# oss0430/SRFRD

Measured on NVIDIA B200. Metric: training seqs/sec; full-catalogue top-10 users/sec, higher is better.
Workload: dtype bf16

## Files before the change

include/srfrd_b200.h:

```cpp
#ifndef SRFRD_B200_H
#define SRFRD_B200_H

#include <stddef.h>
#include <stdint.h>

#ifdef __cplusplus
extern "C" {
#endif

#define SRFRD_ABI_VERSION 10
#if defined(__GNUC__)
#define SRFRD_API __attribute__((visibility("default")))
#else
#define SRFRD_API
#endif

SRFRD_API const char* srfrd_last_error(void);
SRFRD_API int srfrd_abi_version(void);
SRFRD_API int srfrd_device_check(void);

SRFRD_API int srfrd_embed_ln_fwd(const float* item_table, int64_t n_rows, int D, const float* pos_table,
                       const float* aux_table, int64_t n_aux, int F, int mode, const int64_t* seq,
                       const int64_t* aux_ids, int64_t B, int L, float item_scale, const float* ln_w,
                       const float* ln_b, float eps, void* x0_bf16, float* x0_f32, void* q_bf16, float* stats,
                       int ldx, float drop_p, uint64_t drop_seed, uint32_t drop_stream, const float* drop_step,
                       void* stream);

SRFRD_API int srfrd_srfu_labels(const int64_t* fake_ids, int64_t B, int L, int kind, int64_t* labels, void* stream);

SRFRD_API int srfrd_embed_bwd(const void* dx0_bf16, int ldx, const int64_t* seq, const int64_t* aux_ids, int64_t B, int L,
                    int D, int F, int mode, float item_scale, float* d_item, float* d_aux, void* stream);

SRFRD_API int srfrd_layernorm_fwd(const void* x_bf16, int ldx, const float* w, const float* b, float eps, void* y_bf16,
                        float* y_f32, int ldy, float* stats, int64_t T, int H, int64_t row_stride,
                        int64_t row_offset, void* stream);
SRFRD_API int srfrd_layernorm_bwd(const void* dy_bf16, const float* dy_f32, int lddy, const void* x_bf16, int ldx,
                        const float* stats, const float* w, const void* add_bf16, int ldadd,
                        const int64_t* row_ids, void* dx_bf16, int lddx, float* dw, float* db, int64_t T, int H,
                        void* stream);

typedef struct {
  const float* bias;
  const void* residual;
  const void* gate;
  const int64_t* row_ids;
  void* out_bf16;
  float* out_f32;
  int ldr, ldg, ldc;
  int relu;
  float drop_p;
  uint32_t drop_stream;
  uint64_t drop_seed;
  const float* drop_step;
  void* ln_out_bf16;
  const float* ln_w;
  const float* ln_b;
  float* ln_stats;
  int ld_ln;
  float ln_eps;
} srfrd_gemm_epilogue_t;

SRFRD_API int srfrd_gemm_tn(const void* A_bf16, int lda, const void* B_bf16, int ldb, int M, int N, int K,
                  const srfrd_gemm_epilogue_t* ep, void* stream);
SRFRD_API int srfrd_gemm_tn_plan(int M, int N, int K, int has_aux, int bf16_out, int fused_ln, int* out);
SRFRD_API int srfrd_gemm_debug_read(long long* host_dst);
SRFRD_API int srfrd_attn_debug_read(long long* host_dst);

SRFRD_API int srfrd_gemm_wgrad(const void* dY_bf16, int lda, const void* X_bf16, int ldb, int64_t T, int Mo, int No,
                     float* dW, int ldw, float* dbias, void* stream);
SRFRD_API int srfrd_gemm_ref(const void* A, int lda, const void* B, int ldb, float* C, int ldc, int M, int N, int K,
                   int a_mn_major, int b_mn_major, void* stream);

SRFRD_API int srfrd_colsum(const void* X_bf16, int64_t M, int N, int64_t ld, float* out, void* stream);
SRFRD_API int srfrd_add_segments(float* in, int64_t n, int seg_in, int seg_out, float* out, void* stream);

SRFRD_API int srfrd_dropout_apply(const void* x_bf16, int ldx, void* out_bf16, int ldo, int64_t M, int N, float drop_p,
                        uint64_t seed, uint32_t stream_id, const float* drop_step, void* stream);

typedef struct {
  const float* src; int src_ld;
  void* dst; int dst_ld;
  void* dst_t; int dst_t_ld;
  int rows, cols;
  int dst_is_f32;
} srfrd_cast_desc_t;
SRFRD_API int srfrd_cast_weights(const srfrd_cast_desc_t* descs_dev, int n, void* stream);
SRFRD_API int srfrd_f32_to_bf16_split(const float* src, int64_t src_ld, const int64_t* row_index, void* hi, void* lo,
                            int64_t rows, int cols, int dst_ld, void* stream);

SRFRD_API int srfrd_attention_fwd(const void* q, int ldq, const void* k, const void* v, int ldkv, void* o, int ldo,
                        float* stats, int64_t B, int L, int H, int heads, float drop_p, uint64_t seed, uint32_t stream_id,
                        const float* drop_step, void* stream);
SRFRD_API int srfrd_attention_bwd(const void* dout, int lddo, const void* q, int ldq, const void* k, const void* v, int ldkv,
                        const void* o, int ldo, float* stats, void* dq, int lddq, void* dk, void* dv, int lddkv, int64_t B,
                        int L, int H, int heads, float drop_p, uint64_t seed, uint32_t stream_id, const float* drop_step,
                        void* stream);

SRFRD_API int srfrd_score_fwd(const float* h, int ldh, const float* item_table, const float* fake_table, const int64_t* pos,
                    const int64_t* neg, const int64_t* prs, const int64_t* nrs, int64_t T, int D, int F, float* zp,
                    float* zn, void* stream);
SRFRD_API int srfrd_score_bwd(const float* h, int ldh, const float* item_table, const float* fake_table, const int64_t* pos,
                    const int64_t* neg, const int64_t* prs, const int64_t* nrs, const float* dzp, const float* dzn,
                    int64_t T, int D, int F, float* dh, int lddh, float* d_item, float* d_fake, void* stream);
SRFRD_API int srfrd_score_loss_fused(const float* h, int ldh, const float* item_table, const float* fake_table,
                           const int64_t* pos, const int64_t* neg, const int64_t* prs, const int64_t* nrs,
                           const float* w_pos, const float* w_neg, const float* norm, int64_t T, int D, int F,
                           float* zp, float* zn, float* loss_acc, float* dh, int lddh, float* d_item, float* d_fake,
                           void* stream);
SRFRD_API int srfrd_weight_sums(const int64_t* pos, const float* w_pos, const float* w_neg, int64_t T, float* out2,
                      void* stream);
SRFRD_API int srfrd_loss_finalize(float* acc2, const float* norm2, float* loss, void* stream);

SRFRD_API int srfrd_adam_tick(float* state3, float beta1, float beta2, void* stream);
SRFRD_API int srfrd_adam_step(float* p, float* g, float* m, float* v, int64_t n, float lr, float beta1, float beta2, float eps,
                    const float* state3, int zero_grad, void* stream);

SRFRD_API int srfrd_adam_step_fused(float* p, float* g, float* m, float* v, int64_t n, float lr, float beta1, float beta2,
                          float eps, float* state8, int zero_grad, float* acc2, const float* norm2, float* loss,
                          void* stream, const int64_t* l2_seg, int l2_n_seg, const float* l2_coef, const float* l2_reg);

SRFRD_API int srfrd_param_l2_plan(const int64_t* seg_host, int n_seg, int64_t* n_chunks);
SRFRD_API int srfrd_param_l2(const float* p, const int64_t* seg, int n_seg, int64_t n_chunks, float l2, float* coef,
                   float* reg, double* ws, void* stream);

#define SRFRD_TOPK_KMAX 64
SRFRD_API int srfrd_catalogue_topk_plan(int64_t U, int64_t n_rows, int64_t row_lo, int D, int n_split, int* chunks_out,
                                        int k);
SRFRD_API int srfrd_catalogue_topk_kmax(int D, int n_split, int* kmax_out);
SRFRD_API int srfrd_catalogue_topk(const void* feats_bf16, int64_t U, int64_t u_pad, int n_split, const void* table_bf16,
                         int64_t n_rows, int64_t row_lo, int64_t id_base, int D, int ld_feats, int ld_table,
                         int chunks, float* part_scores, int* part_ids, float* packed_out, void* stream, int k);
SRFRD_API int srfrd_merge_topk(const float* scores, const int* ids, int64_t U, int nlists, int k, float* out_scores,
                     int64_t* out_ids, void* stream);
SRFRD_API int srfrd_merge_topk_packed(const float* packed, int64_t U, int nlists, int k, float* out_scores,
                            int64_t* out_ids, void* stream);
SRFRD_API int srfrd_catalogue_rank(const void* feats_bf16, int64_t U, int64_t u_pad, int n_split,
                                   const void* table_bf16, int64_t n_rows, int64_t row_lo, int64_t id_base,
                                   int D, int ld_feats, int ld_table,
                                   const void* target_rows_bf16, int ld_target, const int64_t* target_ids,
                                   float* target_scores, int* rank_out, void* stream);

SRFRD_API int srfrd_catalogue_ce_plan(int Dp, int64_t* smem_bytes, int* ring_stages, int* tmem_cols);
SRFRD_API int srfrd_catalogue_ce_fwd(const void* h_bf16, int ldh, const void* table_bf16, int ldt, int64_t n_items, int Dp,
                                     const int64_t* pos, const float* w_pos, const int* row_tok, const int* rows_dev,
                                     int64_t cap_rows, float* lse, float* loss_acc, void* stream);
SRFRD_API int srfrd_catalogue_ce_bwd(const void* h_bf16, int ldh, const void* table_bf16, int ldt, int64_t n_items, int Dp,
                                     int D, const int64_t* pos, const float* w_pos, const float* norm, const int* row_tok,
                                     const int* rows_dev, int64_t cap_rows, const float* lse, float* dh, int lddh,
                                     float* d_item, int ldd, void* stream);

SRFRD_API int srfrd_sample_batch(const int64_t* offsets, const int* items, const int8_t* labels, const float* p_fake,
                       const int* eligible, int n_eligible, int itemnum, int B, int L, int policy, uint64_t seed,
                       const float* step, int64_t* users, int64_t* seq, int64_t* rsq, int64_t* pos, int64_t* prs,
                       int64_t* neg, int64_t* nrs, float* w_pos, void* stream);

SRFRD_API int srfrd_sample_candidates(const int64_t* offsets, const int* items, const int* users0, const int* target,
                            int64_t U, int itemnum, int C, uint64_t seed, int64_t* cand, void* stream);
SRFRD_API int srfrd_candidate_rank(const float* feats, int ldf, const float* item_table, int64_t n_rows, int D,
                         const int64_t* cand, int64_t U, int C, const float* fake_table, int F,
                         const int64_t* user_label, float* logits, int ldl, int* rank, int* err_flag, void* stream);
SRFRD_API int srfrd_add_user_term(float* logits, int ldl, int64_t U, int I, const float* feats_tail, int ldf,
                        const float* fake_table, const int64_t* label, int F, void* stream);

typedef struct {
  int* rows;
  int* cnt;
  int* seq_first;
  int* tok_row;
  int* row_tok;
  int64_t* row_ids;
  int* row_info;
  int* tile_row0;
  int* last_row;
  int64_t cap;
} srfrd_pack_t;
SRFRD_API int srfrd_pack_plan(const int64_t* seq, const int64_t* keep, int64_t B, int L, const srfrd_pack_t* pk, void* stream);
SRFRD_API int srfrd_set_row_limit(const int* rows_dev);
SRFRD_API int srfrd_embed_ln_fwd_packed(const float* item_table, int64_t n_rows, int D, const float* pos_table,
                              const float* aux_table, int64_t n_aux, int F, int mode, const int64_t* seq,
                              const int64_t* aux_ids, int64_t B, int L, float item_scale, const float* ln_w,
                              const float* ln_b, float eps, void* x0_bf16, void* q_bf16, float* stats, int ldx,
                              float drop_p, uint64_t drop_seed, uint32_t drop_stream, const float* drop_step,
                              const int* row_tok, const int* rows_dev, int64_t cap_rows, void* stream);
SRFRD_API int srfrd_layernorm_fwd_rows(const void* x_bf16, int ldx, const float* w, const float* b, float eps, float* y_f32,
                             int ldy, const int* row_index, int64_t n, int H, void* stream);
SRFRD_API int srfrd_attention_packed_supported(int L, int H, int heads);
SRFRD_API int srfrd_attention_packed_oproj_supported(int L, int H, int heads);
SRFRD_API int srfrd_attention_fwd_packed(const void* q, int ldq, const void* k, const void* v, int ldkv, void* o, int ldo,
                               const srfrd_pack_t* pk, int L, int H, int heads, float drop_p, uint64_t seed,
                               uint32_t stream_id, const float* drop_step, void* stream, const void* wo, int ldw,
                               const float* bo, const void* res, int ldres, const float* ln_w, const float* ln_b,
                               float ln_eps, float* ln_stats, void* r, int ldr, void* y, int ldy);
SRFRD_API int srfrd_attention_bwd_packed(const void* dout, int lddo, const void* q, int ldq, const void* k, const void* v,
                               int ldkv, void* dq, int lddq, void* dk, void* dv, int lddkv, const srfrd_pack_t* pk,
                               int L, int H, int heads, float drop_p, uint64_t seed, uint32_t stream_id,
                               const float* drop_step, void* stream, const void* dr, int lddr, const void* woT, int ldw);
SRFRD_API int srfrd_score_loss_fused_packed(const float* h, int ldh, const float* item_table, const float* fake_table,
                                  const int64_t* pos, const int64_t* neg, const int64_t* prs, const int64_t* nrs,
                                  const float* w_pos, const float* w_neg, const float* norm, int D, int F,
                                  float* loss_acc, float* dh, int lddh, float* d_item, float* d_fake,
                                  const int* row_tok, const int* rows_dev, int64_t cap_rows, void* stream);
SRFRD_API int srfrd_embed_bwd_packed(const void* dx0_bf16, int ldx, const int64_t* seq, const int64_t* aux_ids,
                           const int* row_tok, const int* rows_dev, int64_t cap_rows, int L, int D, int F, int mode,
                           float item_scale, float* d_item, float* d_aux, float* d_pos, void* stream);

typedef struct {
  const float* bias1; const float* bias2;
  const void* gate; int ldg;
  int relu1;
  float drop1_p, drop2_p; uint32_t drop1_stream, drop2_stream; uint64_t drop_seed; const float* drop_step;
  const void* residual; int ldr;
  int residual_is_a;
  const int64_t* row_ids;
  void* mid_out; int ldm;
  void* out; int ldc;
  void* ln_out; int ld_ln; const float* ln_w; const float* ln_b; float* ln_stats; float ln_eps;
} srfrd_mlp2_t;
SRFRD_API int srfrd_mlp2_tn(const void* A_bf16, int lda, const void* W1_bf16, int ldw1, const void* W2_bf16, int ldw2, int M, int N,
                  const srfrd_mlp2_t* ep, void* stream);

SRFRD_API int srfrd_attention_live_items(const int* tok_row, int64_t B, int L, int heads, int* q_lo, int* items, int* n_live,
                               void* stream);
SRFRD_API int srfrd_set_attention_live(const int* q_lo, const int* items, const int* n_live, const int* tok_row);

typedef struct {
  const void* src; int ld_s;
  void* dst; int ld_d;
  int W;
  int mode;
} srfrd_repack_part_t;
SRFRD_API int srfrd_unpack_rows(const srfrd_repack_part_t* parts, int n_parts, const srfrd_pack_t* pk, int64_t B, int L,
                      void* stream);
SRFRD_API int srfrd_pack_rows(const srfrd_repack_part_t* parts, int n_parts, const srfrd_pack_t* pk, int64_t B, int L,
                    void* stream);

SRFRD_API int srfrd_dp_adam_step(float* const* grad_ptrs_dev, float* const* param_ptrs_dev, uint32_t* const* signal_ptrs_dev,
                       int rank, int world, int64_t n, float* m, float* v, float lr, float beta1, float beta2, float eps,
                       float* state8, const float* norm2, uint32_t* local4, void* stream, const int64_t* l2_seg,
                       int l2_n_seg, const float* l2_coef, const float* l2_reg);

#ifdef __cplusplus
}
#endif
#endif
```

srfrd_b200/_lib.py:

```python
from __future__ import annotations

import ctypes as C
import os

_HERE = os.path.dirname(os.path.abspath(__file__))
LIB_PATH = os.environ.get("SRFRD_B200_LIB") or os.path.join(_HERE, "lib", "libsrfrd_b200.so")

vp, i32, i64, f32, u32, u64 = C.c_void_p, C.c_int, C.c_int64, C.c_float, C.c_uint32, C.c_uint64


class GemmEpilogue(C.Structure):
    _fields_ = [("bias", vp), ("residual", vp), ("gate", vp), ("row_ids", vp), ("out_bf16", vp), ("out_f32", vp),
                ("ldr", i32), ("ldg", i32), ("ldc", i32), ("relu", i32), ("drop_p", f32), ("drop_stream", u32),
                ("drop_seed", u64), ("drop_step", vp),
                ("ln_out_bf16", vp), ("ln_w", vp), ("ln_b", vp), ("ln_stats", vp), ("ld_ln", i32), ("ln_eps", f32)]


class CastDesc(C.Structure):
    _fields_ = [("src", vp), ("src_ld", i32), ("dst", vp), ("dst_ld", i32), ("dst_t", vp), ("dst_t_ld", i32),
                ("rows", i32), ("cols", i32), ("dst_is_f32", i32)]


class Mlp2Epilogue(C.Structure):
    _fields_ = [("bias1", vp), ("bias2", vp), ("gate", vp), ("ldg", i32), ("relu1", i32), ("drop1_p", f32), ("drop2_p", f32),
                ("drop1_stream", u32), ("drop2_stream", u32), ("drop_seed", u64), ("drop_step", vp), ("residual", vp), ("ldr", i32),
                ("residual_is_a", i32), ("row_ids", vp), ("mid_out", vp), ("ldm", i32), ("out", vp), ("ldc", i32),
                ("ln_out", vp), ("ld_ln", i32), ("ln_w", vp), ("ln_b", vp), ("ln_stats", vp), ("ln_eps", f32)]


class PackDesc(C.Structure):
    _fields_ = [("rows", vp), ("cnt", vp), ("seq_first", vp), ("tok_row", vp), ("row_tok", vp), ("row_ids", vp),
                ("row_info", vp), ("tile_row0", vp), ("last_row", vp), ("cap", i64)]


class RepackPart(C.Structure):
    _fields_ = [("src", vp), ("ld_s", i32), ("dst", vp), ("ld_d", i32), ("W", i32), ("mode", i32)]


SIGNATURES = {
    "srfrd_abi_version": [],
    "srfrd_device_check": [],
    "srfrd_embed_ln_fwd": [vp, i64, i32, vp, vp, i64, i32, i32, vp, vp, i64, i32, f32, vp, vp, f32, vp, vp, vp, vp, i32,
                           f32, u64, u32, vp, vp],
    "srfrd_srfu_labels": [vp, i64, i32, i32, vp, vp],
    "srfrd_embed_bwd": [vp, i32, vp, vp, i64, i32, i32, i32, i32, f32, vp, vp, vp],
    "srfrd_layernorm_fwd": [vp, i32, vp, vp, f32, vp, vp, i32, vp, i64, i32, i64, i64, vp],
    "srfrd_layernorm_bwd": [vp, vp, i32, vp, i32, vp, vp, vp, i32, vp, vp, i32, vp, vp, i64, i32, vp],
    "srfrd_gemm_tn": [vp, i32, vp, i32, i32, i32, i32, C.POINTER(GemmEpilogue), vp],
    "srfrd_mlp2_tn": [vp, i32, vp, i32, vp, i32, i32, i32, C.POINTER(Mlp2Epilogue), vp],
    "srfrd_gemm_tn_plan": [i32, i32, i32, i32, i32, i32, vp],
    "srfrd_gemm_debug_read": [vp],
    "srfrd_attn_debug_read": [vp],
    "srfrd_gemm_wgrad": [vp, i32, vp, i32, i64, i32, i32, vp, i32, vp, vp],
    "srfrd_gemm_ref": [vp, i32, vp, i32, vp, i32, i32, i32, i32, i32, i32, vp],
    "srfrd_colsum": [vp, i64, i32, i64, vp, vp],
    "srfrd_add_segments": [vp, i64, i32, i32, vp, vp],
    "srfrd_dropout_apply": [vp, i32, vp, i32, i64, i32, f32, u64, u32, vp, vp],
    "srfrd_cast_weights": [vp, i32, vp],
    "srfrd_f32_to_bf16_split": [vp, i64, vp, vp, vp, i64, i32, i32, vp],
    "srfrd_attention_fwd": [vp, i32, vp, vp, i32, vp, i32, vp, i64, i32, i32, i32, f32, u64, u32, vp, vp],
    "srfrd_attention_bwd": [vp, i32, vp, i32, vp, vp, i32, vp, i32, vp, vp, i32, vp, vp, i32, i64, i32, i32, i32, f32, u64,
                            u32, vp, vp],
    "srfrd_score_fwd": [vp, i32, vp, vp, vp, vp, vp, vp, i64, i32, i32, vp, vp, vp],
    "srfrd_score_bwd": [vp, i32, vp, vp, vp, vp, vp, vp, vp, vp, i64, i32, i32, vp, i32, vp, vp, vp],
    "srfrd_score_loss_fused": [vp, i32, vp, vp, vp, vp, vp, vp, vp, vp, vp, i64, i32, i32, vp, vp, vp, vp, i32, vp, vp, vp],
    "srfrd_weight_sums": [vp, vp, vp, i64, vp, vp],
    "srfrd_loss_finalize": [vp, vp, vp, vp],
    "srfrd_adam_tick": [vp, f32, f32, vp],
    "srfrd_adam_step": [vp, vp, vp, vp, i64, f32, f32, f32, f32, vp, i32, vp],
    "srfrd_adam_step_fused": [vp, vp, vp, vp, i64, f32, f32, f32, f32, vp, i32, vp, vp, vp, vp, vp, i32, vp, vp],
    "srfrd_param_l2_plan": [C.POINTER(i64), i32, C.POINTER(i64)],
    "srfrd_param_l2": [vp, vp, i32, i64, f32, vp, vp, vp, vp],
    "srfrd_catalogue_topk_plan": [i64, i64, i64, i32, i32, C.POINTER(i32), i32],
    "srfrd_catalogue_topk_kmax": [i32, i32, C.POINTER(i32)],
    "srfrd_catalogue_topk": [vp, i64, i64, i32, vp, i64, i64, i64, i32, i32, i32, i32, vp, vp, vp, vp, i32],
    "srfrd_merge_topk_packed": [vp, i64, i32, i32, vp, vp, vp],
    "srfrd_catalogue_rank": [vp, i64, i64, i32, vp, i64, i64, i64, i32, i32, i32, vp, i32, vp, vp, vp, vp],
    "srfrd_catalogue_ce_plan": [i32, C.POINTER(i64), C.POINTER(i32), C.POINTER(i32)],
    "srfrd_catalogue_ce_fwd": [vp, i32, vp, i32, i64, i32, vp, vp, vp, vp, i64, vp, vp, vp],
    "srfrd_catalogue_ce_bwd": [vp, i32, vp, i32, i64, i32, i32, vp, vp, vp, vp, vp, i64, vp, vp, i32, vp, i32, vp],
    "srfrd_attention_live_items": [vp, i64, i32, i32, vp, vp, vp, vp],
    "srfrd_set_attention_live": [vp, vp, vp, vp],
    "srfrd_merge_topk": [vp, vp, i64, i32, i32, vp, vp, vp],
    "srfrd_unpack_rows": [C.POINTER(RepackPart), i32, C.POINTER(PackDesc), i64, i32, vp],
    "srfrd_pack_rows": [C.POINTER(RepackPart), i32, C.POINTER(PackDesc), i64, i32, vp],
    "srfrd_dp_adam_step": [vp, vp, vp, i32, i32, i64, vp, vp, f32, f32, f32, f32, vp, vp, vp, vp, vp, i32, vp, vp],
    "srfrd_pack_plan": [vp, vp, i64, i32, C.POINTER(PackDesc), vp],
    "srfrd_set_row_limit": [vp],
    "srfrd_embed_ln_fwd_packed": [vp, i64, i32, vp, vp, i64, i32, i32, vp, vp, i64, i32, f32, vp, vp, f32, vp, vp, vp, i32,
                                  f32, u64, u32, vp, vp, vp, i64, vp],
    "srfrd_layernorm_fwd_rows": [vp, i32, vp, vp, f32, vp, i32, vp, i64, i32, vp],
    "srfrd_attention_packed_supported": [i32, i32, i32],
    "srfrd_attention_packed_oproj_supported": [i32, i32, i32],
    "srfrd_attention_fwd_packed": [vp, i32, vp, vp, i32, vp, i32, C.POINTER(PackDesc), i32, i32, i32, f32, u64, u32, vp, vp,
                                   vp, i32, vp, vp, i32, vp, vp, f32, vp, vp, i32, vp, i32],
    "srfrd_attention_bwd_packed": [vp, i32, vp, i32, vp, vp, i32, vp, i32, vp, vp, i32, C.POINTER(PackDesc), i32, i32, i32,
                                   f32, u64, u32, vp, vp, vp, i32, vp, i32],
    "srfrd_score_loss_fused_packed": [vp, i32, vp, vp, vp, vp, vp, vp, vp, vp, vp, i32, i32, vp, vp, i32, vp, vp, vp, vp,
                                      i64, vp],
    "srfrd_embed_bwd_packed": [vp, i32, vp, vp, vp, vp, i64, i32, i32, i32, i32, f32, vp, vp, vp, vp],
    "srfrd_sample_candidates": [vp, vp, vp, vp, i64, i32, i32, u64, vp, vp],
    "srfrd_candidate_rank": [vp, i32, vp, i64, i32, vp, i64, i32, vp, i32, vp, vp, i32, vp, vp, vp],
    "srfrd_add_user_term": [vp, i32, i64, i32, vp, i32, vp, vp, i32, vp],
    "srfrd_sample_batch": [vp, vp, vp, vp, vp, i32, i32, i32, i32, i32, u64, vp, vp, vp, vp, vp, vp, vp, vp, vp, vp],
}

_lib = None
_device_ok = False
launch_count = 0


def load() -> C.CDLL:
    global _lib
    if _lib is not None:
        return _lib
    if not os.path.exists(LIB_PATH):
        raise RuntimeError(
            f"srfrd_b200: {LIB_PATH} is not built. Run `make -C srfrd_b200/csrc` (needs nvcc, sm_100a). "
            "There is no CPU fallback.")
    lib = C.CDLL(LIB_PATH)
    lib.srfrd_last_error.restype = C.c_char_p
    lib.srfrd_last_error.argtypes = []
    for name, argtypes in SIGNATURES.items():
        fn = getattr(lib, name)
        fn.argtypes = argtypes
        fn.restype = C.c_int
    if lib.srfrd_abi_version() != 10:
        raise RuntimeError("srfrd_b200: ABI version mismatch between _lib.py and the built library")
    _lib = lib
    return lib


def require_device() -> None:
    global _device_ok
    if _device_ok:
        return
    lib = load()
    if lib.srfrd_device_check() != 0:
        raise RuntimeError("srfrd_b200: " + lib.srfrd_last_error().decode())
    _device_ok = True


_profile = None


def set_profile(records) -> None:
    global _profile
    _profile = records


def call(name: str, *args) -> None:
    global launch_count
    lib = _lib or load()
    if _profile is not None:
        import torch
        e0, e1 = torch.cuda.Event(enable_timing=True), torch.cuda.Event(enable_timing=True)
        e0.record()
        rc = getattr(lib, name)(*args)
        e1.record()
        _profile.append((name, args, e0, e1))
    else:
        rc = getattr(lib, name)(*args)
    if rc != 0:
        raise RuntimeError(f"{name}: {lib.srfrd_last_error().decode()}")
    launch_count += 1
```

srfrd_b200/csrc/loss_scatter_adam.cu:

```cuda
#include "common.cuh"
#include "srfrd_b200.h"

namespace srfrd {

static constexpr int MAXC = 16;

struct ScoreParams {
  const float* h; int ldh;
  const float* item_table;
  const float* fake_table;
  const int64_t *pos, *neg, *prs, *nrs;
  const float *w_pos, *w_neg;
  const float* norm;
  const float *dzp_in, *dzn_in;
  float *zp, *zn;
  float* loss_acc;
  float* dh; int lddh;
  float* d_item; float* d_fake;
  int64_t T; int D, F;
  int mode;
  const int* row_tok;
  const int* rows_dev;
  int group;
};

__device__ __forceinline__ float softplus(float x) { return fmaxf(x, 0.f) + log1pf(__expf(-fabsf(x))); }
__device__ __forceinline__ float sigmoidf(float x) { return 1.f / (1.f + __expf(-x)); }

template <int NC>
__global__ void __launch_bounds__(256, (NC <= 9 ? 2 : 1)) score_kernel(ScoreParams p) {
  __shared__ float red[2][8];
  pdl_prologue_done();
  const int lane = threadIdx.x & 31, warp = threadIdx.x >> 5, nw = blockDim.x >> 5;
  const int64_t warp0 = (int64_t)blockIdx.x * nw + warp, nwarps = (int64_t)gridDim.x * nw;
  const int W = p.D + (p.fake_table ? p.F : 0);
  float lp_acc = 0.f, ln_acc = 0.f;
  float inv_np = 0.f, inv_nn = 0.f;
  if (p.mode == 1) {
    const float a = __ldg(p.norm), b = __ldg(p.norm + 1);
    inv_np = a > 0.f ? 1.f / a : 0.f;
    inv_nn = b > 0.f ? 1.f / b : 0.f;
  }
  float fk1[NC], fk2[NC];
#pragma unroll
  for (int i = 0; i < NC; ++i) fk1[i] = fk2[i] = 0.f;
  const bool dh_vec = p.dh && (p.lddh == W) && (W % 4 == 0) && ((reinterpret_cast<uintptr_t>(p.dh) & 15) == 0);
  if (p.rows_dev) p.T = min(p.T, (int64_t)__ldg(p.rows_dev));
  const int G = p.group;
  for (int64_t t0 = warp0 * G; t0 < p.T; t0 += nwarps * G) {
    const int64_t tl = t0 + lane;
    bool in = lane < G && tl < p.T;
    int my_tok = 0;
    if (p.row_tok && in) { my_tok = __ldg(p.row_tok + tl); in = my_tok >= 0; }
    const int64_t my_src = p.row_tok ? (int64_t)my_tok : tl;
    int64_t my_pid = 0, my_nid = 0, my_pf = 0, my_nf = 0;
    float my_a = 0.f, my_b = 0.f;
    bool my_active = false;
    if (in) {
      my_pid = __ldg(p.pos + my_src);
      my_nid = __ldg(p.neg + my_src);
      if (p.mode == 1) {
        my_a = p.w_pos ? __ldg(p.w_pos + my_src) : (my_pid != 0 ? 1.f : 0.f);
        my_b = p.w_neg ? __ldg(p.w_neg + my_src) : my_a;
        my_active = (my_a != 0.f) || (my_b != 0.f) || p.zp;
      } else if (p.mode == 2) {
        my_a = __ldg(p.dzp_in + my_src);
        my_b = __ldg(p.dzn_in + my_src);
        my_active = (my_a != 0.f) || (my_b != 0.f);
      } else {
        my_active = true;
      }
      if (p.fake_table && my_active) { my_pf = __ldg(p.prs + my_src); my_nf = __ldg(p.nrs + my_src); }
    }
    unsigned mask = __ballot_sync(0xffffffffu, my_active);
    if (p.dh) {
      const int nrow = (int)min((int64_t)G, p.T - t0);
      if (dh_vec) {
        const int per_row = W >> 2, total = nrow * per_row;
        float4* base = reinterpret_cast<float4*>(p.dh + t0 * p.lddh);
        for (int i = lane; i < total; i += 32)
          if (!((mask >> (i / per_row)) & 1u)) base[i] = make_float4(0.f, 0.f, 0.f, 0.f);
      } else {
        for (int r = 0; r < nrow; ++r) {
          if ((mask >> r) & 1u) continue;
          for (int c = lane; c < W; c += 32) p.dh[(t0 + r) * p.lddh + c] = 0.f;
        }
      }
    }
    struct Tok {
      int64_t t, tsrc, pid, nid; int pf, nf; float ta, tb;
      float hv[NC], ep[NC], en[NC];
    };
    auto fetch = [&](Tok& k, int r) {
      k.t = t0 + r;
      k.tsrc = p.row_tok ? (int64_t)__shfl_sync(0xffffffffu, my_tok, r) : k.t;
      k.pid = __shfl_sync(0xffffffffu, my_pid, r); k.nid = __shfl_sync(0xffffffffu, my_nid, r);
      k.pf = (int)__shfl_sync(0xffffffffu, (int)my_pf, r); k.nf = (int)__shfl_sync(0xffffffffu, (int)my_nf, r);
      k.ta = __shfl_sync(0xffffffffu, my_a, r); k.tb = __shfl_sync(0xffffffffu, my_b, r);
#pragma unroll
      for (int i = 0; i < NC; ++i) {
        const int c = lane + 32 * i;
        k.hv[i] = k.ep[i] = k.en[i] = 0.f;
        if (c < W) {
          k.hv[i] = p.h[k.t * p.ldh + c];
          if (c < p.D) {
            k.ep[i] = __ldg(p.item_table + k.pid * p.D + c);
            k.en[i] = __ldg(p.item_table + k.nid * p.D + c);
          } else {
            k.ep[i] = __ldg(p.fake_table + (int64_t)k.pf * p.F + (c - p.D));
            k.en[i] = __ldg(p.fake_table + (int64_t)k.nf * p.F + (c - p.D));
          }
        }
      }
    };
    auto finish = [&](const Tok& k) {
      float sp = 0.f, sn = 0.f;
#pragma unroll
      for (int i = 0; i < NC; ++i) { sp = fmaf(k.hv[i], k.ep[i], sp); sn = fmaf(k.hv[i], k.en[i], sn); }
      const float zp = warp_sum(sp), zn = warp_sum(sn);
      if (p.zp && lane == 0) { p.zp[k.tsrc] = zp; p.zn[k.tsrc] = zn; }
      if (p.mode == 0) return;
      float dzp = k.ta, dzn = k.tb;
      if (p.mode == 1) {
        lp_acc += k.ta * softplus(-zp);
        ln_acc += k.tb * softplus(zn);
        dzp = k.ta * (sigmoidf(zp) - 1.f) * inv_np;
        dzn = k.tb * sigmoidf(zn) * inv_nn;
      }
#pragma unroll
      for (int i = 0; i < NC; ++i) {
        const int c = lane + 32 * i;
        if (c < W) {
          if (p.dh) p.dh[k.t * p.lddh + c] = dzp * k.ep[i] + dzn * k.en[i];
          if (c < p.D) {
            if (p.d_item && k.pid != 0 && dzp != 0.f) red_add_f32(p.d_item + k.pid * p.D + c, dzp * k.hv[i]);
            if (p.d_item && k.nid != 0 && dzn != 0.f) red_add_f32(p.d_item + k.nid * p.D + c, dzn * k.hv[i]);
          } else {
            const float gp = dzp * k.hv[i], gn = dzn * k.hv[i];
            fk1[i] += (k.pf == 1 ? gp : 0.f) + (k.nf == 1 ? gn : 0.f);
            fk2[i] += (k.pf == 2 ? gp : 0.f) + (k.nf == 2 ? gn : 0.f);
          }
        }
      }
    };
    if (NC <= 4) {
      if (mask) {
        Tok cur, nxt;
        { const int r = __ffs(mask) - 1; mask &= mask - 1; fetch(cur, r); }
        while (true) {
          const bool more = mask != 0;
          if (more) { const int r = __ffs(mask) - 1; mask &= mask - 1; fetch(nxt, r); }
          finish(cur);
          if (!more) break;
          cur = nxt;
        }
      }
    } else {
      while (mask) {
        const int r = __ffs(mask) - 1;
        mask &= mask - 1;
        Tok cur;
        fetch(cur, r);
        finish(cur);
      }
    }
  }
  if (p.d_fake) {
#pragma unroll
    for (int i = 0; i < NC; ++i) {
      const int c = lane + 32 * i;
      if (c >= p.D && c < W) {
        if (fk1[i] != 0.f) red_add_f32(p.d_fake + 1 * p.F + (c - p.D), fk1[i]);
        if (fk2[i] != 0.f) red_add_f32(p.d_fake + 2 * p.F + (c - p.D), fk2[i]);
      }
    }
  }
  if (p.mode == 1 && p.loss_acc) {
    if (lane == 0) { red[0][warp] = lp_acc; red[1][warp] = ln_acc; }
    __syncthreads();
    if (threadIdx.x == 0) {
      float a = 0.f, b = 0.f;
      for (int w = 0; w < nw; ++w) { a += red[0][w]; b += red[1][w]; }
      red_add_f32(p.loss_acc, a);
      red_add_f32(p.loss_acc + 1, b);
    }
  }
}

__global__ void __launch_bounds__(256) weight_sums_kernel(const int64_t* pos, const float* w_pos, const float* w_neg,
                                                          int64_t T, float* out) {
  __shared__ float red[2][8];
  float a = 0.f, b = 0.f;
  for (int64_t t = (int64_t)blockIdx.x * blockDim.x + threadIdx.x; t < T; t += (int64_t)gridDim.x * blockDim.x) {
    const float wp = w_pos ? w_pos[t] : (pos[t] != 0 ? 1.f : 0.f);
    a += wp;
    b += w_neg ? w_neg[t] : wp;
  }
  a = warp_sum(a); b = warp_sum(b);
  const int lane = threadIdx.x & 31, warp = threadIdx.x >> 5;
  if (lane == 0) { red[0][warp] = a; red[1][warp] = b; }
  __syncthreads();
  if (threadIdx.x == 0) {
    a = b = 0.f;
    for (int w = 0; w < (int)(blockDim.x >> 5); ++w) { a += red[0][w]; b += red[1][w]; }
    red_add_f32(out, a);
    red_add_f32(out + 1, b);
  }
}

__global__ void loss_finalize_kernel(float* acc, const float* norm, float* loss) {
  pdl_prologue_done();
  const float a = norm[0] > 0.f ? acc[0] / norm[0] : 0.f;
  const float b = norm[1] > 0.f ? acc[1] / norm[1] : 0.f;
  loss[0] = a + b;
  acc[0] = 0.f; acc[1] = 0.f;
}

struct EmbedBwdParams {
  const bf16* dx0; int ldx;
  const int64_t* seq;
  const int64_t* aux_ids;
  int L, D, F, mode;
  float item_scale;
  float* d_item;
  float* d_aux;
};

__global__ void embed_bwd_kernel(EmbedBwdParams p) {
  extern __shared__ int64_t ids[];
  pdl_prologue_done();
  const int64_t b = blockIdx.x;
  const int c = threadIdx.x;
  const int H = p.D + (p.mode == 1 ? p.F : 0);
  for (int l = threadIdx.x; l < p.L; l += blockDim.x) {
    ids[l] = p.seq[b * p.L + l];
    ids[p.L + l] = (p.mode == 1 && p.aux_ids) ? p.aux_ids[b * p.L + l] : 0;
  }
  __syncthreads();
  if (c >= H) return;
  float acc1 = 0.f, acc2 = 0.f, accu = 0.f;
  for (int l = 0; l < p.L; ++l) {
    const int64_t id = ids[l];
    if (id == 0) continue;
    const float v = bf2f(p.dx0[(b * p.L + l) * p.ldx + c]);
    if (c < p.D) {
      red_add_f32(p.d_item + id * p.D + c, v * p.item_scale);
      accu += v;
    } else {
      const int64_t f = ids[p.L + l];
      if (f == 1) acc1 += v;
      else if (f == 2) acc2 += v;
    }
  }
  if (p.mode == 1 && c >= p.D && p.d_aux) {
    if (acc1 != 0.f) red_add_f32(p.d_aux + 1 * p.F + (c - p.D), acc1);
    if (acc2 != 0.f) red_add_f32(p.d_aux + 2 * p.F + (c - p.D), acc2);
  }
  if (p.mode == 2 && c < p.D && p.d_aux && accu != 0.f)
    red_add_f32(p.d_aux + p.aux_ids[b] * p.D + c, accu);
}

static constexpr int EB_SLICE = 64;
__global__ void __launch_bounds__(512) embed_bwd_packed_kernel(EmbedBwdParams p, const int* row_tok, const int* rows_dev, int64_t cap,
                                                              float* d_pos) {
  extern __shared__ float spos[];
  pdl_prologue_done();
  const int x = threadIdx.x, y = threadIdx.y, RPB = blockDim.y;
  const int c = blockIdx.y * EB_SLICE + x;
  const int H = p.D + (p.mode == 1 ? p.F : 0);
  const int tid = y * blockDim.x + x, nthr = blockDim.x * blockDim.y;
  const bool pos_slice = blockIdx.y * EB_SLICE < p.D;
  if (pos_slice) for (int i = tid; i < p.L * EB_SLICE; i += nthr) spos[i] = 0.f;
  __syncthreads();
  const int64_t M = min(cap, (int64_t)__ldg(rows_dev));
  float acc1 = 0.f, acc2 = 0.f;
  for (int64_t r = (int64_t)blockIdx.x * RPB + y; r < M; r += (int64_t)gridDim.x * RPB) {
    const int tok = __ldg(row_tok + r);
    if (tok < 0 || c >= H) continue;
    const int64_t id = __ldg(p.seq + tok);
    if (id == 0) continue;
    const float v = bf2f(p.dx0[r * p.ldx + c]);
    if (c < p.D) {
      red_add_f32(p.d_item + id * p.D + c, v * p.item_scale);
      atomicAdd(&spos[(tok % p.L) * EB_SLICE + x], v);
      if (p.mode == 2 && p.d_aux) red_add_f32(p.d_aux + p.aux_ids[tok / p.L] * p.D + c, v);
    } else if (p.aux_ids) {
      const int64_t f = __ldg(p.aux_ids + tok);
      if (f == 1) acc1 += v;
      else if (f == 2) acc2 += v;
    }
  }
  if (p.mode == 1 && c >= p.D && c < H && p.d_aux) {
    if (acc1 != 0.f) red_add_f32(p.d_aux + 1 * p.F + (c - p.D), acc1);
    if (acc2 != 0.f) red_add_f32(p.d_aux + 2 * p.F + (c - p.D), acc2);
  }
  __syncthreads();
  if (d_pos && pos_slice)
    for (int i = tid; i < p.L * EB_SLICE; i += nthr) {
      const int l = i / EB_SLICE, cc = blockIdx.y * EB_SLICE + i % EB_SLICE;
      if (cc < p.D && spos[i] != 0.f) red_add_f32(d_pos + l * p.D + cc, spos[i]);
    }
}

__global__ void add_segments_kernel(float* in, int64_t n, int seg_in, int seg_out, float* out) {
  pdl_prologue_done();
  const int64_t i = (int64_t)blockIdx.x * blockDim.x + threadIdx.x;
  if (i >= n) return;
  const int c = (int)(i % seg_in);
  if (c < seg_out) out[(i / seg_in) * seg_out + c] += in[i];
  in[i] = 0.f;
}

__global__ void adam_tick_kernel(float* state, float beta1, float beta2) {
  pdl_prologue_done();
  const float step = state[0] + 1.f;
  state[0] = step;
  state[1] = (float)(1.0 - pow((double)beta1, (double)step));
  state[2] = (float)(1.0 - pow((double)beta2, (double)step));
  state[3] = __uint_as_float(__float_as_uint(state[3]) + 1u);
}

static constexpr int64_t L2_CHUNK = 8192;

__device__ __forceinline__ void l2_chunk_prefix(const int64_t* seg, int n_seg, int64_t* s_c0) {
  const int t = threadIdx.x;
  s_c0[t + 1] = t < n_seg ? (seg[2 * t + 1] + L2_CHUNK - 1) / L2_CHUNK : 0;
  if (t == 0) s_c0[0] = 0;
  __syncthreads();
  for (int d = 1; d < L2_THREADS; d <<= 1) {
    const int64_t a = t >= d ? s_c0[t + 1 - d] : 0;
    __syncthreads();
    s_c0[t + 1] += a;
    __syncthreads();
  }
}

__device__ __forceinline__ double block_sum_f64(double x, double* s_red) {
#pragma unroll
  for (int o = 16; o > 0; o >>= 1) x += __shfl_xor_sync(0xffffffffu, x, o);
  if ((threadIdx.x & 31) == 0) s_red[threadIdx.x >> 5] = x;
  __syncthreads();
  double s = 0.0;
  if (threadIdx.x == 0)
    for (int w = 0; w < L2_THREADS / 32; ++w) s += s_red[w];
  __syncthreads();
  return s;
}

__global__ void __launch_bounds__(L2_THREADS) param_l2_kernel(const float* __restrict__ p, const int64_t* __restrict__ seg,
                                                               int n_seg, int64_t n_chunks, float l2, float* coef, float* reg,
                                                               double* ws) {
  __shared__ int64_t s_c0[L2_THREADS + 1];
  __shared__ double s_red[L2_THREADS / 32];
  __shared__ double s_norm[L2_THREADS];
  __shared__ bool s_last;
  pdl_prologue_done();
  l2_chunk_prefix(seg, n_seg, s_c0);
  double* part = ws + 1;
  for (int64_t c = blockIdx.x; c < n_chunks; c += gridDim.x) {
    int lo = 0, hi = n_seg - 1;
    while (lo < hi) {
      const int mid = (lo + hi + 1) >> 1;
      if (s_c0[mid] <= c) lo = mid; else hi = mid - 1;
    }
    const int64_t off = seg[2 * lo], numel = seg[2 * lo + 1];
    const int64_t b = (c - s_c0[lo]) * L2_CHUNK;
    const int64_t e = min(numel, b + L2_CHUNK);
    const float4* p4 = reinterpret_cast<const float4*>(p + off);
    double acc = 0.0;
#pragma unroll
    for (int k = 0; k < (int)(L2_CHUNK / 4 / L2_THREADS); ++k) {
      const int64_t j = b + 4 * ((int64_t)k * L2_THREADS + threadIdx.x);
      if (j < e) {
        const float4 x = __ldcg(p4 + j / 4);
        const float xs[4] = {x.x, x.y, x.z, x.w};
#pragma unroll
        for (int q = 0; q < 4; ++q)
          if (j + q < e) acc = fma((double)xs[q], (double)xs[q], acc);
      }
    }
    const double s = block_sum_f64(acc, s_red);
    if (threadIdx.x == 0) part[c] = s;
  }
  __threadfence();
  __syncthreads();
  if (threadIdx.x == 0) s_last = atomicAdd(reinterpret_cast<unsigned*>(ws), 1u) == gridDim.x - 1;
  __syncthreads();
  if (!s_last) return;
  __threadfence();
  const int warp = threadIdx.x >> 5, lane = threadIdx.x & 31;
  for (int t = warp; t < n_seg; t += L2_THREADS / 32) {
    double s = 0.0;
    for (int64_t c = s_c0[t] + lane; c < s_c0[t + 1]; c += 32) s += __ldcg(part + c);
#pragma unroll
    for (int o = 16; o > 0; o >>= 1) s += __shfl_xor_sync(0xffffffffu, s, o);
    if (lane == 0) {
      const double nrm = sqrt(s);
      s_norm[t] = nrm;
      coef[t] = nrm > 0.0 ? (float)((double)l2 / nrm) : 0.f;
    }
  }
  __syncthreads();
  if (threadIdx.x == 0) {
    double tot = 0.0;
    for (int t = 0; t < n_seg; ++t) tot += s_norm[t];
    reg[0] = (float)((double)l2 * tot);
    *reinterpret_cast<unsigned*>(ws) = 0u;
  }
}

template <bool L2>
__global__ void __launch_bounds__(256) adam_fused_kernel(float* __restrict__ p, float* __restrict__ g, float* __restrict__ m,
                                                         float* __restrict__ v, int64_t n, float lr, float beta1, float beta2,
                                                         float eps, float* state, int zero_grad, float* acc, const float* norm,
                                                         float* loss, L2Segments l2s) {
  __shared__ float s_bc[2];
  pdl_prologue_done();
  if (threadIdx.x == 0) {
    const float step = state[0] + 1.f;
    s_bc[0] = (float)(1.0 - pow((double)beta1, (double)step));
    s_bc[1] = (float)(1.0 - pow((double)beta2, (double)step));
  }
  if (blockIdx.x == 0 && threadIdx.x == 32 && acc) {
    const float a = norm[0] > 0.f ? acc[0] / norm[0] : 0.f;
    const float b = norm[1] > 0.f ? acc[1] / norm[1] : 0.f;
    if constexpr (L2) loss[0] = a + b + l2s.reg[0];
    else loss[0] = a + b;
    acc[0] = 0.f; acc[1] = 0.f;
  }
  int64_t* s_off = nullptr;
  float* s_coef = nullptr;
  if constexpr (L2) {
    s_off = l2_smem().off;
    s_coef = l2_smem().coef;
    l2_load_starts(l2s, s_off, s_coef);
  }
  __syncthreads();
  const float step_size = lr / s_bc[0];
  const float inv_sqrt_bc2 = rsqrtf(s_bc[1]);
  const int64_t n4 = n >> 2;
  int t = 0;
  if constexpr (L2) t = l2_find(s_off, l2s.n_seg, (int64_t)blockIdx.x * blockDim.x + threadIdx.x);
  for (int64_t i = (int64_t)blockIdx.x * blockDim.x + threadIdx.x; i < n4; i += (int64_t)gridDim.x * blockDim.x) {
    float4 pp = reinterpret_cast<float4*>(p)[i], gg = reinterpret_cast<float4*>(g)[i];
    float4 mm = reinterpret_cast<float4*>(m)[i], vv = reinterpret_cast<float4*>(v)[i];
    float* pa = &pp.x; float* ga = &gg.x; float* ma = &mm.x; float* va = &vv.x;
    if constexpr (L2) {
      t = l2_advance(s_off, l2s.n_seg, t, i);
      const float c = s_coef[t];
#pragma unroll
      for (int j = 0; j < 4; ++j) ga[j] += c * pa[j];
    }
#pragma unroll
    for (int j = 0; j < 4; ++j) {
      ma[j] = beta1 * ma[j] + (1.f - beta1) * ga[j];
      va[j] = beta2 * va[j] + (1.f - beta2) * ga[j] * ga[j];
      pa[j] -= step_size * ma[j] / (sqrtf(va[j]) * inv_sqrt_bc2 + eps);
    }
    reinterpret_cast<float4*>(p)[i] = pp;
    reinterpret_cast<float4*>(m)[i] = mm;
    reinterpret_cast<float4*>(v)[i] = vv;
    if (zero_grad) reinterpret_cast<float4*>(g)[i] = make_float4(0.f, 0.f, 0.f, 0.f);
  }
  if (blockIdx.x == 0 && threadIdx.x < (n & 3)) {
    const int64_t i = (n4 << 2) + threadIdx.x;
    m[i] = beta1 * m[i] + (1.f - beta1) * g[i];
    v[i] = beta2 * v[i] + (1.f - beta2) * g[i] * g[i];
    p[i] -= step_size * m[i] / (sqrtf(v[i]) * inv_sqrt_bc2 + eps);
    if (zero_grad) g[i] = 0.f;
  }
  __syncthreads();
  if (threadIdx.x == 0) {
    int* done = reinterpret_cast<int*>(state + 4);
    if (atomicAdd(done, 1) == (int)gridDim.x - 1) {
      *done = 0;
      state[0] = state[0] + 1.f;
      state[1] = s_bc[0];
      state[2] = s_bc[1];
      state[3] = __uint_as_float(__float_as_uint(state[3]) + 1u);
    }
  }
}

__global__ void __launch_bounds__(256) adam_kernel(float* __restrict__ p, float* __restrict__ g, float* __restrict__ m,
                                                   float* __restrict__ v, int64_t n, float lr, float beta1, float beta2,
                                                   float eps, const float* __restrict__ state, int zero_grad) {
  pdl_prologue_done();
  const float step_size = lr / state[1];
  const float inv_sqrt_bc2 = rsqrtf(state[2]);
  const int64_t n4 = n >> 2;
  for (int64_t i = (int64_t)blockIdx.x * blockDim.x + threadIdx.x; i < n4; i += (int64_t)gridDim.x * blockDim.x) {
    float4 pp = reinterpret_cast<float4*>(p)[i], gg = reinterpret_cast<float4*>(g)[i];
    float4 mm = reinterpret_cast<float4*>(m)[i], vv = reinterpret_cast<float4*>(v)[i];
    float* pa = &pp.x; float* ga = &gg.x; float* ma = &mm.x; float* va = &vv.x;
#pragma unroll
    for (int j = 0; j < 4; ++j) {
      ma[j] = beta1 * ma[j] + (1.f - beta1) * ga[j];
      va[j] = beta2 * va[j] + (1.f - beta2) * ga[j] * ga[j];
      pa[j] -= step_size * ma[j] / (sqrtf(va[j]) * inv_sqrt_bc2 + eps);
    }
    reinterpret_cast<float4*>(p)[i] = pp;
    reinterpret_cast<float4*>(m)[i] = mm;
    reinterpret_cast<float4*>(v)[i] = vv;
    if (zero_grad) reinterpret_cast<float4*>(g)[i] = make_float4(0.f, 0.f, 0.f, 0.f);
  }
  if (blockIdx.x == 0 && threadIdx.x < (n & 3)) {
    const int64_t i = (n4 << 2) + threadIdx.x;
    m[i] = beta1 * m[i] + (1.f - beta1) * g[i];
    v[i] = beta2 * v[i] + (1.f - beta2) * g[i] * g[i];
    p[i] -= step_size * m[i] / (sqrtf(v[i]) * inv_sqrt_bc2 + eps);
    if (zero_grad) g[i] = 0.f;
  }
}

}

using namespace srfrd;

static int score_launch(ScoreParams& p, void* stream) {
  const int W = p.D + (p.fake_table ? p.F : 0);
  SRFRD_REQUIRE(W <= 32 * MAXC, "score: width %d unsupported", W);
  if (p.T == 0) return 0;
  if (p.group != 8) p.group = 32;
  int64_t blocks = (p.T + 8 * p.group - 1) / (8 * p.group);
  const int64_t cap = (int64_t)num_sms() * 8;
  if (blocks > cap) blocks = cap;
  const int nc = (W + 31) / 32;
#define SCORE_CALL(NC) SRFRD_CUDA(launch_pdl(score_kernel<NC>, dim3((unsigned)blocks), dim3(256), 0, (cudaStream_t)stream, p))
  if (nc <= 1) SCORE_CALL(1);
  else if (nc <= 2) SCORE_CALL(2);
  else if (nc <= 3) SCORE_CALL(3);
  else if (nc <= 4) SCORE_CALL(4);
  else if (nc <= 6) SCORE_CALL(6);
  else if (nc <= 9) SCORE_CALL(9);
  else SCORE_CALL(MAXC);
#undef SCORE_CALL
  SRFRD_LAUNCH_CHECK();
  return 0;
}

extern "C" int srfrd_score_fwd(const float* h, int ldh, const float* item_table, const float* fake_table,
                               const int64_t* pos, const int64_t* neg, const int64_t* prs, const int64_t* nrs,
                               int64_t T, int D, int F, float* zp, float* zn, void* stream) {
  SRFRD_REQUIRE(h && item_table && pos && neg && zp && zn, "score_fwd: null pointer");
  SRFRD_REQUIRE(!fake_table || (prs && nrs), "score_fwd: fake ids required with a fake table");
  ScoreParams p = {};
  p.h = h; p.ldh = ldh; p.item_table = item_table; p.fake_table = fake_table; p.pos = pos; p.neg = neg; p.prs = prs;
  p.nrs = nrs; p.T = T; p.D = D; p.F = F; p.zp = zp; p.zn = zn; p.mode = 0;
  return score_launch(p, stream);
}

extern "C" int srfrd_score_bwd(const float* h, int ldh, const float* item_table, const float* fake_table,
                               const int64_t* pos, const int64_t* neg, const int64_t* prs, const int64_t* nrs,
                               const float* dzp, const float* dzn, int64_t T, int D, int F, float* dh, int lddh,
                               float* d_item, float* d_fake, void* stream) {
  SRFRD_REQUIRE(h && item_table && pos && neg && dzp && dzn && dh, "score_bwd: null pointer");
  SRFRD_REQUIRE(!fake_table || (prs && nrs), "score_bwd: fake ids required with a fake table");
  ScoreParams p = {};
  p.h = h; p.ldh = ldh; p.item_table = item_table; p.fake_table = fake_table; p.pos = pos; p.neg = neg; p.prs = prs;
  p.nrs = nrs; p.T = T; p.D = D; p.F = F; p.dzp_in = dzp; p.dzn_in = dzn; p.dh = dh; p.lddh = lddh; p.d_item = d_item;
  p.d_fake = d_fake; p.mode = 2;
  return score_launch(p, stream);
}

extern "C" int srfrd_score_loss_fused(const float* h, int ldh, const float* item_table, const float* fake_table,
                                      const int64_t* pos, const int64_t* neg, const int64_t* prs, const int64_t* nrs,
                                      const float* w_pos, const float* w_neg, const float* norm, int64_t T, int D,
                                      int F, float* zp, float* zn, float* loss_acc, float* dh, int lddh, float* d_item,
                                      float* d_fake, void* stream) {
  SRFRD_REQUIRE(h && item_table && pos && neg && norm && loss_acc, "score_loss_fused: null pointer");
  SRFRD_REQUIRE(!fake_table || (prs && nrs), "score_loss_fused: fake ids required with a fake table");
  SRFRD_REQUIRE((zp == nullptr) == (zn == nullptr), "score_loss_fused: pass both logit outputs or neither");
  ScoreParams p = {};
  p.h = h; p.ldh = ldh; p.item_table = item_table; p.fake_table = fake_table; p.pos = pos; p.neg = neg; p.prs = prs;
  p.nrs = nrs; p.w_pos = w_pos; p.w_neg = w_neg; p.norm = norm; p.T = T; p.D = D; p.F = F; p.zp = zp; p.zn = zn;
  p.loss_acc = loss_acc; p.dh = dh; p.lddh = lddh; p.d_item = d_item; p.d_fake = d_fake; p.mode = 1;
  return score_launch(p, stream);
}

extern "C" int srfrd_score_loss_fused_packed(const float* h, int ldh, const float* item_table, const float* fake_table,
                                             const int64_t* pos, const int64_t* neg, const int64_t* prs, const int64_t* nrs,
                                             const float* w_pos, const float* w_neg, const float* norm, int D, int F,
                                             float* loss_acc, float* dh, int lddh, float* d_item, float* d_fake,
                                             const int* row_tok, const int* rows_dev, int64_t cap_rows, void* stream) {
  SRFRD_REQUIRE(h && item_table && pos && neg && norm && loss_acc && row_tok && rows_dev, "score_loss_fused_packed: null pointer");
  SRFRD_REQUIRE(!fake_table || (prs && nrs), "score_loss_fused_packed: fake ids required with a fake table");
  ScoreParams p = {};
  p.h = h; p.ldh = ldh; p.item_table = item_table; p.fake_table = fake_table; p.pos = pos; p.neg = neg; p.prs = prs;
  p.nrs = nrs; p.w_pos = w_pos; p.w_neg = w_neg; p.norm = norm; p.T = cap_rows; p.D = D; p.F = F;
  p.loss_acc = loss_acc; p.dh = dh; p.lddh = lddh; p.d_item = d_item; p.d_fake = d_fake; p.mode = 1;
  p.row_tok = row_tok; p.rows_dev = rows_dev; p.group = 8;
  return score_launch(p, stream);
}

extern "C" int srfrd_weight_sums(const int64_t* pos, const float* w_pos, const float* w_neg, int64_t T, float* out2,
                                 void* stream) {
  SRFRD_REQUIRE(pos && out2, "weight_sums: null pointer");
  SRFRD_CUDA(cudaMemsetAsync(out2, 0, 2 * sizeof(float), (cudaStream_t)stream));
  if (T == 0) return 0;
  int64_t blocks = (T + 2047) / 2048;
  if (blocks > num_sms() * 2) blocks = num_sms() * 2;
  weight_sums_kernel<<<(unsigned)blocks, 256, 0, (cudaStream_t)stream>>>(pos, w_pos, w_neg, T, out2);
  SRFRD_LAUNCH_CHECK();
  return 0;
}

extern "C" int srfrd_loss_finalize(float* acc2, const float* norm2, float* loss, void* stream) {
  SRFRD_REQUIRE(acc2 && norm2 && loss, "loss_finalize: null pointer");
  SRFRD_CUDA(launch_pdl(loss_finalize_kernel, dim3(1), dim3(1), 0, (cudaStream_t)stream, acc2, norm2, loss));
  SRFRD_LAUNCH_CHECK();
  return 0;
}

extern "C" int srfrd_embed_bwd(const void* dx0, int ldx, const int64_t* seq, const int64_t* aux_ids, int64_t B, int L,
                               int D, int F, int mode, float item_scale, float* d_item, float* d_aux, void* stream) {
  SRFRD_REQUIRE(dx0 && seq && d_item, "embed_bwd: null pointer");
  SRFRD_REQUIRE(mode >= 0 && mode <= 2, "embed_bwd: bad mode");
  SRFRD_REQUIRE(mode != 2 || aux_ids, "embed_bwd: labels required for mode 2");
  const int H = D + (mode == 1 ? F : 0);
  SRFRD_REQUIRE(H <= 1024, "embed_bwd: width %d unsupported", H);
  if (B == 0) return 0;
  EmbedBwdParams p;
  p.dx0 = (const bf16*)dx0; p.ldx = ldx; p.seq = seq; p.aux_ids = aux_ids; p.L = L; p.D = D; p.F = F; p.mode = mode;
  p.item_scale = item_scale; p.d_item = d_item; p.d_aux = d_aux;
  const int threads = (H + 31) & ~31;
  SRFRD_CUDA(launch_pdl(embed_bwd_kernel, dim3((unsigned)B), dim3(threads), 2 * L * sizeof(int64_t), (cudaStream_t)stream, p));
  SRFRD_LAUNCH_CHECK();
  return 0;
}

extern "C" int srfrd_embed_bwd_packed(const void* dx0, int ldx, const int64_t* seq, const int64_t* aux_ids,
                                      const int* row_tok, const int* rows_dev, int64_t cap_rows, int L, int D, int F,
                                      int mode, float item_scale, float* d_item, float* d_aux, float* d_pos, void* stream) {
  SRFRD_REQUIRE(dx0 && seq && d_item && row_tok && rows_dev, "embed_bwd_packed: null pointer");
  SRFRD_REQUIRE(mode >= 0 && mode <= 2, "embed_bwd_packed: bad mode");
  SRFRD_REQUIRE(mode != 2 || aux_ids, "embed_bwd_packed: labels required for mode 2");
  const int H = D + (mode == 1 ? F : 0);
  SRFRD_REQUIRE(H <= 512, "embed_bwd_packed: width %d unsupported", H);
  if (cap_rows == 0) return 0;
  EmbedBwdParams p;
  p.dx0 = (const bf16*)dx0; p.ldx = ldx; p.seq = seq; p.aux_ids = aux_ids; p.L = L; p.D = D; p.F = F; p.mode = mode;
  p.item_scale = item_scale; p.d_item = d_item; p.d_aux = d_aux;
  const int slices = (H + EB_SLICE - 1) / EB_SLICE;
  const int tx = EB_SLICE, ty = 8;
  const size_t smem = (size_t)L * EB_SLICE * sizeof(float);
  SRFRD_REQUIRE(smem <= 200 * 1024, "embed_bwd_packed: L = %d too long for the shared positional accumulator", L);
  static bool attr = false;
  if (!attr) {
    SRFRD_CUDA(cudaFuncSetAttribute(embed_bwd_packed_kernel, cudaFuncAttributeMaxDynamicSharedMemorySize, 200 * 1024));
    attr = true;
  }
  int per_sm = (int)((200 * 1024) / (smem + 1024));
  if (per_sm > 4) per_sm = 4;
  if (per_sm < 1) per_sm = 1;
  int64_t gx = ((int64_t)num_sms() * per_sm + slices - 1) / slices;
  const int64_t need = (cap_rows + ty - 1) / ty;
  if (gx > need) gx = need;
  if (gx < 1) gx = 1;
  const dim3 grid((unsigned)gx, (unsigned)slices);
  SRFRD_CUDA(launch_pdl(embed_bwd_packed_kernel, grid, dim3(tx, ty), smem, (cudaStream_t)stream, p, row_tok, rows_dev, cap_rows,
                        d_pos));
  SRFRD_LAUNCH_CHECK();
  return 0;
}

extern "C" int srfrd_add_segments(float* in, int64_t n, int seg_in, int seg_out, float* out, void* stream) {
  SRFRD_REQUIRE(in && out && seg_in > 0 && seg_out <= seg_in, "add_segments: bad arguments");
  if (n == 0) return 0;
  SRFRD_CUDA(launch_pdl(add_segments_kernel, dim3((unsigned)((n + 255) / 256)), dim3(256), 0, (cudaStream_t)stream, in, n, seg_in,
                        seg_out, out));
  SRFRD_LAUNCH_CHECK();
  return 0;
}

extern "C" int srfrd_adam_tick(float* state3, float beta1, float beta2, void* stream) {
  SRFRD_REQUIRE(state3, "adam_tick: null state");
  SRFRD_CUDA(launch_pdl(adam_tick_kernel, dim3(1), dim3(1), 0, (cudaStream_t)stream, state3, beta1, beta2));
  SRFRD_LAUNCH_CHECK();
  return 0;
}

extern "C" int srfrd_adam_step(float* p, float* g, float* m, float* v, int64_t n, float lr, float beta1, float beta2,
                               float eps, const float* state3, int zero_grad, void* stream) {
  SRFRD_REQUIRE(p && g && m && v && state3, "adam_step: null pointer");
  SRFRD_REQUIRE((((uintptr_t)p | (uintptr_t)g | (uintptr_t)m | (uintptr_t)v) & 15) == 0, "adam_step: buffers must be 16-byte aligned");
  if (n == 0) return 0;
  int64_t blocks = (n / 4 + 255) / 256;
  if (blocks < 1) blocks = 1;
  if (blocks > num_sms() * 8) blocks = num_sms() * 8;
  SRFRD_CUDA(launch_pdl(adam_kernel, dim3((unsigned)blocks), dim3(256), 0, (cudaStream_t)stream, p, g, m, v, n, lr, beta1, beta2,
                        eps, state3, zero_grad));
  SRFRD_LAUNCH_CHECK();
  return 0;
}

extern "C" int srfrd_adam_step_fused(float* p, float* g, float* m, float* v, int64_t n, float lr, float beta1, float beta2,
                                     float eps, float* state8, int zero_grad, float* acc2, const float* norm2, float* loss,
                                     void* stream, const int64_t* l2_seg, int l2_n_seg, const float* l2_coef,
                                     const float* l2_reg) {
  SRFRD_REQUIRE(p && g && m && v && state8, "adam_step_fused: null pointer");
  SRFRD_REQUIRE(!acc2 || (norm2 && loss), "adam_step_fused: the loss read-out needs norm and loss");
  SRFRD_REQUIRE((((uintptr_t)p | (uintptr_t)g | (uintptr_t)m | (uintptr_t)v) & 15) == 0, "adam_step_fused: buffers must be 16-byte aligned");
  const bool l2 = l2_seg != nullptr;
  SRFRD_REQUIRE(!l2 || (l2_coef && l2_reg && acc2), "adam_step_fused: the l2 term needs coef, reg and the loss read-out");
  SRFRD_REQUIRE(!l2 || (l2_n_seg >= 1 && l2_n_seg <= L2_THREADS && n % 4 == 0),
                "adam_step_fused: l2 needs 1..%d segments and n a multiple of 4", L2_THREADS);
  int64_t blocks = (n / 4 + 255) / 256;
  if (blocks < 1) blocks = 1;
  if (blocks > num_sms() * 8) blocks = num_sms() * 8;
  const L2Segments l2s{l2_seg, l2_n_seg, l2_coef, l2_reg};
  if (l2)
    SRFRD_CUDA(launch_pdl(adam_fused_kernel<true>, dim3((unsigned)blocks), dim3(256), 0, (cudaStream_t)stream, p, g, m, v, n,
                          lr, beta1, beta2, eps, state8, zero_grad, acc2, norm2, loss, l2s));
  else
    SRFRD_CUDA(launch_pdl(adam_fused_kernel<false>, dim3((unsigned)blocks), dim3(256), 0, (cudaStream_t)stream, p, g, m, v, n,
                          lr, beta1, beta2, eps, state8, zero_grad, acc2, norm2, loss, l2s));
  SRFRD_LAUNCH_CHECK();
  return 0;
}

extern "C" int srfrd_param_l2_plan(const int64_t* seg_host, int n_seg, int64_t* n_chunks) {
  SRFRD_REQUIRE(seg_host && n_chunks, "param_l2_plan: null pointer");
  SRFRD_REQUIRE(n_seg >= 1 && n_seg <= L2_THREADS, "param_l2_plan: %d segments (1..%d supported)", n_seg, L2_THREADS);
  int64_t c = 0, end = 0;
  for (int t = 0; t < n_seg; ++t) {
    const int64_t off = seg_host[2 * t], numel = seg_host[2 * t + 1];
    SRFRD_REQUIRE(off % 4 == 0 && off >= end && numel >= 0, "param_l2_plan: segment %d must start 4-aligned after the last", t);
    end = off + numel;
    c += (numel + L2_CHUNK - 1) / L2_CHUNK;
  }
  *n_chunks = c;
  return 0;
}

extern "C" int srfrd_param_l2(const float* p, const int64_t* seg, int n_seg, int64_t n_chunks, float l2, float* coef,
                              float* reg, double* ws, void* stream) {
  SRFRD_REQUIRE(p && seg && coef && reg && ws, "param_l2: null pointer");
  SRFRD_REQUIRE(((uintptr_t)p & 15) == 0, "param_l2: the parameter buffer must be 16-byte aligned");
  SRFRD_REQUIRE(n_seg >= 1 && n_seg <= L2_THREADS && n_chunks >= 0, "param_l2: bad segment / chunk count");
  int64_t grid = n_chunks < 1 ? 1 : n_chunks;
  if (grid > num_sms() * 8) grid = num_sms() * 8;
  SRFRD_CUDA(launch_pdl(param_l2_kernel, dim3((unsigned)grid), dim3(L2_THREADS), 0, (cudaStream_t)stream, p, seg, n_seg,
                        n_chunks, l2, coef, reg, ws));
  SRFRD_LAUNCH_CHECK();
  return 0;
}
```

srfrd_b200/engine.py:

```python
from __future__ import annotations

import math
import os
from contextlib import contextmanager, nullcontext
from dataclasses import dataclass
from typing import Dict, List, Optional, Tuple

import torch

from . import ops

bf16 = torch.bfloat16
LN_EPS = 1e-8

KINDS = ("SRFR", "SRFRN", "SRFU_B", "SRFU_F", "SRFU_R", "SASRec")


@dataclass
class ModelSpec:
    kind: str
    item_number: int
    max_len: int
    D: int
    F: int = 0
    n_labels: int = 0
    num_blocks: int = 2
    num_heads: int = 1
    dropout: float = 0.0

    def __post_init__(self):
        if self.kind not in KINDS:
            raise ValueError(f"unknown model kind {self.kind}")
        if self.H % self.num_heads:
            raise ValueError("hidden size must be divisible by num_heads")
        if (self.H // self.num_heads) % 2:
            raise ValueError(f"srfrd_b200: head width {self.H // self.num_heads} must be even (bf16 pairs)")

    @property
    def H(self) -> int:
        return self.D + self.F if self.kind in ("SRFR", "SRFRN") else self.D

    @property
    def Dout(self) -> int:
        return self.H if self.kind == "SRFRN" else self.D

    @property
    def Hp(self) -> int:
        return (self.H + 15) // 16 * 16

    @property
    def Dp(self) -> int:
        return (self.D + 15) // 16 * 16

    @property
    def Doutp(self) -> int:
        return self.Hp if self.kind == "SRFRN" else self.Dp

    @property
    def padded(self) -> bool:
        return self.Hp != self.H or self.Dp != self.D

    @property
    def mode(self) -> int:
        return 1 if self.kind in ("SRFR", "SRFRN") else (2 if self.kind.startswith("SRFU") else 0)

    @property
    def item_scale(self) -> float:
        return float(self.D ** 0.5) if self.kind == "SASRec" else 1.0

    @property
    def item_key(self) -> str:
        return "item_emb.weight" if self.kind == "SASRec" else "embedding_layer.item_embed.weight"

    @property
    def pos_key(self) -> str:
        return "pos_emb.weight" if self.kind == "SASRec" else "embedding_layer.pos_embed.weight"

    @property
    def aux_key(self) -> Optional[str]:
        if self.mode == 1:
            return "embedding_layer.fake_embed.weight"
        if self.mode == 2:
            return "embedding_layer.user_label_embed.weight"
        return None

    def param_shapes(self) -> List[Tuple[str, Tuple[int, ...]]]:
        H, D, L, N = self.H, self.D, self.max_len, self.item_number
        out: List[Tuple[str, Tuple[int, ...]]] = []
        if self.kind == "SASRec":
            out += [("item_emb.weight", (N + 1, D)), ("pos_emb.weight", (L, D))]
        elif self.mode == 1:
            out += [("embedding_layer.item_embed.weight", (N + 1, D)),
                    ("embedding_layer.fake_embed.weight", (3, self.F)),
                    ("embedding_layer.pos_embed.weight", (L, D))]
        else:
            out += [("embedding_layer.item_embed.weight", (N + 1, D)),
                    ("embedding_layer.user_label_embed.weight", (self.n_labels, D)),
                    ("embedding_layer.pos_embed.weight", (L, D))]
        for i in range(self.num_blocks):
            out += [(f"attention_layernorms.{i}.weight", (H,)), (f"attention_layernorms.{i}.bias", (H,))]
        for i in range(self.num_blocks):
            out += [(f"attention_layers.{i}.in_proj_weight", (3 * H, H)), (f"attention_layers.{i}.in_proj_bias", (3 * H,)),
                    (f"attention_layers.{i}.out_proj.weight", (H, H)), (f"attention_layers.{i}.out_proj.bias", (H,))]
        for i in range(self.num_blocks):
            out += [(f"forward_layernorms.{i}.weight", (H,)), (f"forward_layernorms.{i}.bias", (H,))]
        for i in range(self.num_blocks):
            out += [(f"forward_layers.{i}.conv1.weight", (H, H, 1)), (f"forward_layers.{i}.conv1.bias", (H,)),
                    (f"forward_layers.{i}.conv2.weight", (H, H, 1)), (f"forward_layers.{i}.conv2.bias", (H,))]
        if self.kind == "SRFR":
            out += [("last_conv.weight", (D, H, 1)), ("last_conv.bias", (D,))]
        out += [("last_layernorm.weight", (self.Dout,)), ("last_layernorm.bias", (self.Dout,))]
        return out


class FlatParams:

    def __init__(self, spec: ModelSpec, device, alloc=None):
        self.spec = spec
        self.offsets: Dict[str, Tuple[int, Tuple[int, ...]]] = {}
        off = 0
        for name, shape in spec.param_shapes():
            n = int(math.prod(shape))
            self.offsets[name] = (off, shape)
            off += (n + 3) // 4 * 4
        self.numel = off
        zeros = (lambda n: alloc(n).zero_()) if alloc is not None else (lambda n: torch.zeros(n, dtype=torch.float32, device=device))
        self.data_ext = zeros(off + 4)
        self.data = self.data_ext[:off]
        self.data_tail = self.data_ext[off:]
        self.grad_bucket = zeros(off + 4)
        self.grad = self.grad_bucket[:off]
        self.grad_tail = self.grad_bucket[off:]

    def segments(self) -> List[Tuple[int, int]]:
        return [(off, int(math.prod(shape))) for off, shape in self.offsets.values()]

    def view(self, name: str, grad: bool = False) -> torch.Tensor:
        off, shape = self.offsets[name]
        buf = self.grad if grad else self.data
        return buf[off:off + int(math.prod(shape))].view(shape)

    def mat(self, name: str, grad: bool = False) -> torch.Tensor:
        v = self.view(name, grad)
        return v.view(v.shape[0], -1)


class HotPath:

    def __init__(self, spec: ModelSpec, params: FlatParams):
        self.spec, self.P = spec, params
        self.device = params.data.device
        self._ws_tokens = 0
        self._ws: Dict[str, torch.Tensor] = {}
        self.ws_generation = 0
        self.fwd_version = 0
        self.host_drop_counter = 0
        self._build_shadows()
        self.step_state = torch.zeros(8, dtype=torch.float32, device=self.device)
        self.side = torch.cuda.Stream(device=self.device)
        self.side2 = torch.cuda.Stream(device=self.device)
        self.overlap = os.environ.get("SRFRD_OVERLAP", "1") != "0"
        self.drop_seed = 0x5EED5EED
        self.saved: Optional[dict] = None
        self._plans: Dict[Tuple[int, int], ops.PackedPlan] = {}
        self.packed_default = os.environ.get("SRFRD_PACKED", "1") != "0"
        self.fuse_ffn = os.environ.get("SRFRD_FUSE_FFN", "1") != "0"

    def _build_shadows(self):
        s, P, dev = self.spec, self.P, self.device
        H, D, Hp, Dp = s.H, s.D, s.Hp, s.Dp
        self.sh: Dict[str, torch.Tensor] = {}
        self.vsh: Dict[str, torch.Tensor] = {}
        entries = []
        zb = lambda r, c: torch.zeros(r, c, dtype=bf16, device=dev)

        def vec(name, src, n_pad, dst_off=0, dst=None):
            if not s.padded:
                return
            if dst is None:
                dst = self.vsh.setdefault(name, torch.zeros(n_pad, dtype=torch.float32, device=dev))
            entries.append((src.view(1, -1), dst[dst_off:dst_off + src.numel()].view(1, -1), None))

        for i in range(s.num_blocks):
            win = P.mat(f"attention_layers.{i}.in_proj_weight")
            bin_ = P.view(f"attention_layers.{i}.in_proj_bias")
            self.sh[f"wq{i}"] = zb(Hp, Hp)
            self.sh[f"wkv{i}"] = zb(2 * Hp, Hp)
            self.sh[f"wqT{i}"] = zb(Hp, Hp)
            self.sh[f"wkvT{i}"] = zb(Hp, 2 * Hp)
            entries.append((win[:H], self.sh[f"wq{i}"][:H, :H], self.sh[f"wqT{i}"][:H, :H]))
            entries.append((win[H:2 * H], self.sh[f"wkv{i}"][:H, :H], self.sh[f"wkvT{i}"][:H, :H]))
            entries.append((win[2 * H:], self.sh[f"wkv{i}"][Hp:Hp + H, :H], self.sh[f"wkvT{i}"][:H, Hp:Hp + H]))
            vec(f"bq{i}", bin_[:H], Hp)
            vec(f"bkv{i}", bin_[H:2 * H], 2 * Hp)
            vec(f"bkv{i}", bin_[2 * H:], 2 * Hp, dst_off=Hp)
            for tag, key in (("wo", f"attention_layers.{i}.out_proj"), ("w1", f"forward_layers.{i}.conv1"),
                             ("w2", f"forward_layers.{i}.conv2")):
                self.sh[f"{tag}{i}"] = zb(Hp, Hp)
                self.sh[f"{tag}T{i}"] = zb(Hp, Hp)
                entries.append((P.mat(key + ".weight"), self.sh[f"{tag}{i}"][:H, :H], self.sh[f"{tag}T{i}"][:H, :H]))
                vec(f"b{tag[1]}{i}", P.view(key + ".bias"), Hp)
        if s.kind == "SRFR":
            self.sh["wc"] = zb(Dp, Hp)
            self.sh["wcT"] = zb(Hp, Dp)
            entries.append((P.mat("last_conv.weight"), self.sh["wc"][:D, :H], self.sh["wcT"][:H, :D]))
            vec("bc", P.view("last_conv.bias"), Dp)
        self._cast_entries = entries
        self._cast_table, self._cast_n = ops.make_cast_table(entries, dev)
        self.shadows_version = -1

    def enable_ce_table(self) -> torch.Tensor:
        if "ce_table" not in self.sh:
            s = self.spec
            E = self.P.view(s.item_key)
            self.sh["ce_table"] = torch.zeros(E.shape[0], s.Dp, dtype=bf16, device=self.device)
            for r0 in range(0, E.shape[0], 4096):
                self._cast_entries.append((E[r0:r0 + 4096], self.sh["ce_table"][r0:r0 + 4096, :s.D], None))
            self._cast_table, self._cast_n = ops.make_cast_table(self._cast_entries, self.device)
            self.refresh_shadows()
        return self.sh["ce_table"]

    def bias(self, tag: str, i: Optional[int] = None) -> torch.Tensor:
        s, P = self.spec, self.P
        if s.padded:
            return self.vsh[tag if i is None else f"{tag}{i}"]
        if tag == "bq":
            return P.view(f"attention_layers.{i}.in_proj_bias")[:s.H]
        if tag == "bkv":
            return P.view(f"attention_layers.{i}.in_proj_bias")[s.H:]
        if tag == "bc":
            return P.view("last_conv.bias")
        key = {"bo": f"attention_layers.{i}.out_proj.bias", "b1": f"forward_layers.{i}.conv1.bias",
               "b2": f"forward_layers.{i}.conv2.bias"}[tag]
        return P.view(key)

    def refresh_shadows(self):
        ops.cast_weights(self._cast_table, self._cast_n)

    @contextmanager
    def _branch(self, second: bool = False):
        if not self.overlap:
            yield
            return
        main = torch.cuda.current_stream()
        st = self.side2 if second else self.side
        st.wait_stream(main)
        with torch.cuda.stream(st):
            yield

    def _join(self, second: bool = False):
        if self.overlap:
            torch.cuda.current_stream().wait_stream(self.side2 if second else self.side)

    def _workspace(self, T: int, L: int) -> Dict[str, torch.Tensor]:
        if T <= self._ws_tokens:
            return self._ws
        s, dev = self.spec, self.device
        Lmax = max(L, s.max_len)
        H, nb = s.Hp, s.num_blocks
        ws: Dict[str, torch.Tensor] = {}

        def act(name, w=H, dtype=bf16):
            ws[name] = torch.zeros(T, w, dtype=dtype, device=dev)

        for i in range(nb + 1):
            act(f"x{i}")
        for i in range(nb):
            for n in ("Q", "q", "o", "r", "y", "h1"):
                act(f"{n}{i}")
            act(f"kv{i}", 2 * H)
            act(f"st1_{i}", 2, torch.float32)
            act(f"st2_{i}", 2, torch.float32)
            if Lmax > 128:
                ws[f"ast{i}"] = torch.zeros(T * s.num_heads, 4, dtype=torch.float32, device=dev)
        if s.kind == "SRFR":
            act("c", s.Dp)
        act("stF", 2, torch.float32)
        act("hfin", s.Doutp, torch.float32)
        act("dh", s.Doutp, torch.float32)
        for n in ("gA", "gC", "gD", "gX"):
            act(n)
        for i in range(nb):
            for n in ("gda1_", "gdr_", "gdq_"):
                act(f"{n}{i}")
            act(f"gdz_{i}")
            act(f"gdkv_{i}", 2 * H)
        if s.kind == "SRFR":
            act("gc", s.Dp)
        if s.dropout > 0:
            for i in range(nb):
                act(f"gE_{i}")
        ws["pos_tmp"] = torch.zeros(Lmax * H, dtype=torch.float32, device=dev)
        self._ws, self._ws_tokens = ws, T
        self.ws_generation += 1
        return ws

    def packed_ok(self, B: int, L: int) -> bool:
        return self.packed_mode(B, L) is not None

    def packed_mode(self, B: int, L: int) -> Optional[str]:
        s = self.spec
        if s.padded or s.H % 16 or s.D % 8 or B > 16384 or B < 1:
            return None
        if ops.attention_packed_supported(L, s.H, s.num_heads):
            return "tile"
        if os.environ.get("SRFRD_HYBRID", "1") != "0" and L <= 4096:
            return "hybrid"
        return None

    def _hybrid_ws(self, Td: int) -> Dict[str, torch.Tensor]:
        hw = getattr(self, "_hws", None)
        if hw is not None and hw["_rows"] >= Td:
            return hw
        s, dev = self.spec, self.device
        Hp = s.Hp
        hw = {"_rows": Td}
        z = lambda w: torch.zeros(Td, w, dtype=bf16, device=dev)
        for i in range(s.num_blocks):
            hw[f"qd{i}"], hw[f"kvd{i}"], hw[f"od{i}"] = z(Hp), z(2 * Hp), z(Hp)
        hw["dod"], hw["dqd"], hw["dkvd"] = z(Hp), z(Hp), z(2 * Hp)
        self._hws = hw
        self.ws_generation += 1
        return hw

    def _live_tiles(self, B: int, L: int) -> "ops.LiveTiles":
        key = (B, L)
        lt = getattr(self, "_lives", None)
        if lt is None:
            lt = self._lives = {}
        if key not in lt:
            if len(lt) >= 4:
                lt.clear()
                self.ws_generation += 1
            lt[key] = ops.LiveTiles(B, L, self.spec.num_heads, self.device)
        return lt[key]

    def _plan(self, B: int, L: int) -> "ops.PackedPlan":
        key = (B, L)
        if key not in self._plans:
            if len(self._plans) >= 4:
                self._plans.clear()
                self.ws_generation += 1
            self._plans[key] = ops.PackedPlan(B, L, self.device)
        return self._plans[key]

    def forward(self, seq: torch.Tensor, fake_ids: Optional[torch.Tensor], training: bool,
                last_only: bool = False, save: Optional[bool] = None, packed: bool = False,
                keep: Optional[torch.Tensor] = None) -> torch.Tensor:
        s, P = self.spec, self.P
        B, L = seq.shape
        if L > s.max_len:
            raise RuntimeError(f"sequence length {L} exceeds max_len {s.max_len} (pos_embed rows, SRFR_model.py:12)")
        if packed:
            return self._forward_packed(seq, fake_ids, training, last_only, save, keep)
        T, H, Hp, nb = B * L, s.H, s.Hp, s.num_blocks
        ws = self._workspace(T, L)
        self.fwd_version += 1
        p_drop = s.dropout if training else 0.0
        step = self.step_state[3:4] if p_drop > 0 else None
        seed = (self.drop_seed + self.host_drop_counter * 0x9E3779B97F4A7C15) & 0xFFFFFFFFFFFFFFFF
        seq = seq.contiguous()
        aux_ids = None
        if s.mode == 1:
            aux_ids = None if fake_ids is None else fake_ids.contiguous()
        elif s.mode == 2:
            aux_ids = torch.empty(B, dtype=torch.int64, device=self.device)
            ops.srfu_labels(fake_ids.contiguous(), {"SRFU_B": 0, "SRFU_F": 1, "SRFU_R": 2}[s.kind], aux_ids)
            need = {"SRFU_B": 3, "SRFU_F": L + 1, "SRFU_R": 11}[s.kind]
            if s.n_labels < need and B > 0 and int(aux_ids.max()) >= s.n_labels:
                raise IndexError(f"index out of range in self: {s.kind} user label {int(aux_ids.max())} needs "
                                 f"number_of_labels >= {need}, got {s.n_labels}")
        aux_table = P.view(s.aux_key) if s.aux_key else None
        x = [ws[f"x{i}"][:T] for i in range(nb + 1)]
        ops.embed_ln_fwd(P.view(s.item_key), P.view(s.pos_key), aux_table, s.mode, seq, aux_ids, s.item_scale,
                         P.view("attention_layernorms.0.weight"), P.view("attention_layernorms.0.bias"), LN_EPS,
                         x0_bf16=x[0], q_bf16=ws["Q0"][:T], stats=ws["st1_0"][:T],
                         drop_p=p_drop if s.kind == "SASRec" else 0.0, drop_seed=seed, drop_stream=1, drop_step=step)
        seq_flat = seq.view(-1)
        fuse_ln = (H == Hp) and Hp <= 128 and os.environ.get("SRFRD_FUSE_LN", "1") != "0"
        for i in range(nb):
            Q, q, kv, o, r, y, h1 = (ws[f"{n}{i}"][:T] for n in ("Q", "q", "kv", "o", "r", "y", "h1"))
            with self._branch():
                ops.gemm_tn(x[i], self.sh[f"wkv{i}"], out_bf16=kv, bias=self.bias("bkv", i))
            if i > 0 and not fuse_ln:
                ops.layernorm_fwd(x[i], P.view(f"attention_layernorms.{i}.weight"), P.view(f"attention_layernorms.{i}.bias"),
                                  LN_EPS, y_bf16=Q, stats=ws[f"st1_{i}"][:T], H=H)
            ops.gemm_tn(Q, self.sh[f"wq{i}"], out_bf16=q, bias=self.bias("bq", i))
            self._join()
            ops.attention_fwd(q, kv[:, :Hp], kv[:, Hp:], o, B, L, H, s.num_heads, p_drop, seed, 10 + 4 * i, step,
                              stats=ws.get(f"ast{i}"))
            if fuse_ln:
                ops.gemm_tn(o, self.sh[f"wo{i}"], out_bf16=r, bias=self.bias("bo", i), residual=Q, ln_out=y,
                            ln_w=P.view(f"forward_layernorms.{i}.weight"), ln_b=P.view(f"forward_layernorms.{i}.bias"),
                            ln_eps=LN_EPS, ln_stats=ws[f"st2_{i}"][:T])
            else:
                ops.gemm_tn(o, self.sh[f"wo{i}"], out_bf16=r, bias=self.bias("bo", i), residual=Q)
                ops.layernorm_fwd(r, P.view(f"forward_layernorms.{i}.weight"), P.view(f"forward_layernorms.{i}.bias"), LN_EPS,
                                  y_bf16=y, stats=ws[f"st2_{i}"][:T], H=H)
            ops.gemm_tn(y, self.sh[f"w1{i}"], out_bf16=h1, bias=self.bias("b1", i), relu=True,
                        drop_p=p_drop, drop_seed=seed, drop_stream=11 + 4 * i, drop_step=step)
            nxt = {}
            if fuse_ln and i + 1 < nb:
                nxt = dict(ln_out=ws[f"Q{i + 1}"][:T], ln_w=P.view(f"attention_layernorms.{i + 1}.weight"),
                           ln_b=P.view(f"attention_layernorms.{i + 1}.bias"), ln_eps=LN_EPS, ln_stats=ws[f"st1_{i + 1}"][:T])
            ops.gemm_tn(h1, self.sh[f"w2{i}"], out_bf16=x[i + 1], bias=self.bias("b2", i),
                        residual=y, row_ids=seq_flat, drop_p=p_drop, drop_seed=seed, drop_stream=12 + 4 * i, drop_step=step,
                        **nxt)
        fin_in = x[nb]
        if s.kind == "SRFR":
            ops.gemm_tn(x[nb], self.sh["wc"], out_bf16=ws["c"][:T], bias=self.bias("bc"))
            fin_in = ws["c"][:T]
        hfin = ws["hfin"][:T]
        if last_only:
            out = ws["hfin"][:B]
            ops.layernorm_fwd(fin_in, P.view("last_layernorm.weight"), P.view("last_layernorm.bias"), LN_EPS, y_f32=out,
                              T=B, H=s.Dout, row_stride=L, row_offset=L - 1)
            return out[:, :s.Dout]
        ops.layernorm_fwd(fin_in, P.view("last_layernorm.weight"), P.view("last_layernorm.bias"), LN_EPS, y_f32=hfin,
                          stats=ws["stF"][:T], H=s.Dout)
        if training if save is None else save:
            self.saved = dict(seq=seq, aux_ids=aux_ids, B=B, L=L, p_drop=p_drop, seed=seed, step=step,
                              version=self.fwd_version)
        return hfin.view(B, L, s.Doutp)[..., :s.Dout]

    def backward(self, dh: torch.Tensor, version: Optional[int] = None) -> None:
        s, P, sv = self.spec, self.P, self.saved
        if sv is None:
            raise RuntimeError("backward() without a training forward()")
        if sv["version"] != self.fwd_version or (version is not None and version != sv["version"]):
            raise RuntimeError("srfrd_b200: backward() of a stale forward -- another forward() (training, validation or "
                               "predict) ran on this model after the one being back-propagated and overwrote the shared "
                               "activation workspace; run backward() before the next forward()")
        if sv.get("plan") is not None:
            return self._backward_packed(dh)
        B, L = sv["B"], sv["L"]
        T, H, Hp, nb = B * L, s.H, s.Hp, s.num_blocks
        ws = self._ws
        seq_flat = sv["seq"].view(-1)
        p_drop, seed, step = sv["p_drop"], sv["seed"], sv["step"]
        gA, gC, gD, gX = (ws[n][:T] for n in ("gA", "gC", "gD", "gX"))
        G = lambda name: P.view(name, grad=True)
        GM = lambda name: P.mat(name, grad=True)
        x = [ws[f"x{i}"][:T] for i in range(nb + 1)]
        dz_top = ws[f"gdz_{nb - 1}"][:T]

        if s.kind == "SRFR":
            gc = ws["gc"][:T]
            ops.layernorm_bwd(dh, ws["c"][:T], ws["stF"][:T], P.view("last_layernorm.weight"), gc,
                              G("last_layernorm.weight"), G("last_layernorm.bias"), H=s.D)
            with self._branch():
                ops.gemm_wgrad(gc, x[nb], GM("last_conv.weight"), G("last_conv.bias"), Mo=s.D, No=H)
            ops.gemm_tn(gc, self.sh["wcT"], out_bf16=dz_top, row_ids=seq_flat)
        else:
            ops.layernorm_bwd(dh, x[nb], ws["stF"][:T], P.view("last_layernorm.weight"), dz_top,
                              G("last_layernorm.weight"), G("last_layernorm.bias"), row_ids=seq_flat, H=s.Dout)

        for i in reversed(range(nb)):
            Q, q, kv, o, r, y, h1 = (ws[f"{n}{i}"][:T] for n in ("Q", "q", "kv", "o", "r", "y", "h1"))
            dz, da1, dr, dq, dkv = (ws[f"{n}{i}"][:T] for n in ("gdz_", "gda1_", "gdr_", "gdq_", "gdkv_"))
            dx_out = ws[f"gdz_{i - 1}"][:T] if i > 0 else gA
            dz2 = dz
            if p_drop > 0:
                dz2 = ws[f"gE_{i}"][:T]
                ops.dropout_apply(dz, dz2, Hp, p_drop, seed, 12 + 4 * i, step)
            with self._branch():
                ops.gemm_wgrad(dz2, h1, GM(f"forward_layers.{i}.conv2.weight"), G(f"forward_layers.{i}.conv2.bias"), Mo=H, No=H)
            ops.gemm_tn(dz2, self.sh[f"w2T{i}"], out_bf16=da1, gate=h1, drop_p=p_drop, drop_seed=seed,
                        drop_stream=11 + 4 * i, drop_step=step)
            with self._branch():
                ops.gemm_wgrad(da1, y, GM(f"forward_layers.{i}.conv1.weight"), G(f"forward_layers.{i}.conv1.bias"), Mo=H, No=H)
            ops.gemm_tn(da1, self.sh[f"w1T{i}"], out_bf16=gC, residual=dz)
            ops.layernorm_bwd(gC, r, ws[f"st2_{i}"][:T], P.view(f"forward_layernorms.{i}.weight"), dr,
                              G(f"forward_layernorms.{i}.weight"), G(f"forward_layernorms.{i}.bias"), H=H)
            with self._branch():
                ops.gemm_wgrad(dr, o, GM(f"attention_layers.{i}.out_proj.weight"), G(f"attention_layers.{i}.out_proj.bias"),
                               Mo=H, No=H)
            ops.gemm_tn(dr, self.sh[f"woT{i}"], out_bf16=gC)
            ops.attention_bwd(gC, q, kv[:, :Hp], kv[:, Hp:], dq, dkv[:, :Hp], dkv[:, Hp:], B, L, H, s.num_heads, p_drop,
                              seed, 10 + 4 * i, step, o=o, stats=ws.get(f"ast{i}"))
            gin = GM(f"attention_layers.{i}.in_proj_weight")
            gbin = G(f"attention_layers.{i}.in_proj_bias")
            with self._branch():
                ops.gemm_wgrad(dq, Q, gin[:H], gbin[:H], Mo=H, No=H)
                if Hp == H:
                    ops.gemm_wgrad(dkv, x[i], gin[H:], gbin[H:], Mo=2 * H, No=H)
                else:
                    ops.gemm_wgrad(dkv[:, :Hp], x[i], gin[H:2 * H], gbin[H:2 * H], Mo=H, No=H)
                    ops.gemm_wgrad(dkv[:, Hp:], x[i], gin[2 * H:], gbin[2 * H:], Mo=H, No=H)
            with self._branch(second=True):
                ops.gemm_tn(dkv, self.sh[f"wkvT{i}"], out_bf16=gX)
            ops.gemm_tn(dq, self.sh[f"wqT{i}"], out_bf16=gD, residual=dr)
            self._join(second=True)
            ops.layernorm_bwd(gD, x[i], ws[f"st1_{i}"][:T], P.view(f"attention_layernorms.{i}.weight"), dx_out,
                              G(f"attention_layernorms.{i}.weight"), G(f"attention_layernorms.{i}.bias"),
                              add=gX, row_ids=seq_flat, H=H)

        dx0 = gA
        if s.kind == "SASRec" and p_drop > 0:
            ops.dropout_apply(gA, gC, H, p_drop, seed, 1, step)
            dx0 = gC
        aux_grad = G(s.aux_key) if s.aux_key else None
        ops.embed_bwd(dx0, sv["seq"], sv["aux_ids"], s.D, s.F if s.mode == 1 else 0, s.mode, s.item_scale,
                      G(s.item_key), aux_grad)
        pos_tmp = ws["pos_tmp"][:L * Hp]
        ops.colsum(dx0, pos_tmp, M=B, N=L * Hp, ld=L * Hp)
        ops.add_segments(pos_tmp, L * Hp, Hp, s.D, G(s.pos_key))
        self._join()
        self.saved = None

    def _forward_packed(self, seq, fake_ids, training, last_only, save, keep):
        s, P = self.spec, self.P
        B, L = seq.shape
        H, Hp, nb = s.H, s.Hp, s.num_blocks
        plan = self._plan(B, L)
        T = plan.cap
        ws = self._workspace(T, L)
        self.fwd_version += 1
        p_drop = s.dropout if training else 0.0
        step = self.step_state[3:4] if p_drop > 0 else None
        seed = (self.drop_seed + self.host_drop_counter * 0x9E3779B97F4A7C15) & 0xFFFFFFFFFFFFFFFF
        seq = seq.contiguous()
        aux_ids = None
        if s.mode == 1:
            aux_ids = None if fake_ids is None else fake_ids.contiguous()
        elif s.mode == 2:
            aux_ids = torch.empty(B, dtype=torch.int64, device=self.device)
            ops.srfu_labels(fake_ids.contiguous(), {"SRFU_B": 0, "SRFU_F": 1, "SRFU_R": 2}[s.kind], aux_ids)
            need = {"SRFU_B": 3, "SRFU_F": L + 1, "SRFU_R": 11}[s.kind]
            if s.n_labels < need and int(aux_ids.max()) >= s.n_labels:
                raise IndexError(f"index out of range in self: {s.kind} user label {int(aux_ids.max())} needs "
                                 f"number_of_labels >= {need}, got {s.n_labels}")
        aux_table = P.view(s.aux_key) if s.aux_key else None
        plan.build(seq, None if keep is None else keep.contiguous())
        hyb = self._hybrid_ws(B * L) if self.packed_mode(B, L) == "hybrid" else None
        live = None
        if hyb is not None and os.environ.get("SRFRD_LIVE_TILES", "1") != "0":
            live = self._live_tiles(B, L)
            live.build(plan)
        x = [ws[f"x{i}"][:T] for i in range(nb + 1)]
        row_ids = plan.row_ids
        fuse_ln = Hp <= 128 and os.environ.get("SRFRD_FUSE_LN", "1") != "0"
        fuse_oproj = self._fuse_oproj(hyb, L, fuse_ln) & 1
        with ops.row_limit(plan.rows):
            ops.embed_ln_fwd_packed(P.view(s.item_key), P.view(s.pos_key), aux_table, s.mode, seq, aux_ids, s.item_scale,
                                    P.view("attention_layernorms.0.weight"), P.view("attention_layernorms.0.bias"), LN_EPS,
                                    x[0], ws["Q0"][:T], ws["st1_0"][:T], plan,
                                    drop_p=p_drop if s.kind == "SASRec" else 0.0, drop_seed=seed, drop_stream=1, drop_step=step)
            for i in range(nb):
                Q, q, kv, o, r, y, h1 = (ws[f"{n}{i}"][:T] for n in ("Q", "q", "kv", "o", "r", "y", "h1"))
                with self._branch():
                    ops.gemm_tn(x[i], self.sh[f"wkv{i}"], out_bf16=kv, bias=self.bias("bkv", i))
                if i > 0 and not fuse_ln:
                    ops.layernorm_fwd(x[i], P.view(f"attention_layernorms.{i}.weight"), P.view(f"attention_layernorms.{i}.bias"),
                                      LN_EPS, y_bf16=Q, stats=ws[f"st1_{i}"][:T], H=H)
                ops.gemm_tn(Q, self.sh[f"wq{i}"], out_bf16=q, bias=self.bias("bq", i))
                self._join()
                if fuse_oproj:
                    ops.attention_fwd_packed(q, kv[:, :Hp], kv[:, Hp:], o, plan, L, H, s.num_heads, p_drop, seed, 10 + 4 * i, step,
                                             wo=self.sh[f"wo{i}"], bias=self.bias("bo", i), residual=Q, r=r, y=y,
                                             ln_w=P.view(f"forward_layernorms.{i}.weight"),
                                             ln_b=P.view(f"forward_layernorms.{i}.bias"), ln_eps=LN_EPS,
                                             ln_stats=ws[f"st2_{i}"][:T])
                elif hyb is None:
                    ops.attention_fwd_packed(q, kv[:, :Hp], kv[:, Hp:], o, plan, L, H, s.num_heads, p_drop, seed, 10 + 4 * i, step)
                else:
                    qd, kvd, od = hyb[f"qd{i}"][:B * L], hyb[f"kvd{i}"][:B * L], hyb[f"od{i}"][:B * L]
                    ops.unpack_rows([(q, qd, Hp, 0), (kv, kvd, 2 * Hp, 0)], plan)
                    with (live.active() if live is not None else nullcontext()):
                        ops.attention_fwd(qd, kvd[:, :Hp], kvd[:, Hp:], od, B, L, H, s.num_heads, p_drop, seed, 10 + 4 * i, step,
                                          stats=ws.get(f"ast{i}"))
                    ops.pack_rows([(od, o, Hp, 0)], plan)
                if fuse_oproj:
                    pass
                elif fuse_ln:
                    ops.gemm_tn(o, self.sh[f"wo{i}"], out_bf16=r, bias=self.bias("bo", i), residual=Q, ln_out=y,
                                ln_w=P.view(f"forward_layernorms.{i}.weight"), ln_b=P.view(f"forward_layernorms.{i}.bias"),
                                ln_eps=LN_EPS, ln_stats=ws[f"st2_{i}"][:T])
                else:
                    ops.gemm_tn(o, self.sh[f"wo{i}"], out_bf16=r, bias=self.bias("bo", i), residual=Q)
                    ops.layernorm_fwd(r, P.view(f"forward_layernorms.{i}.weight"), P.view(f"forward_layernorms.{i}.bias"),
                                      LN_EPS, y_bf16=y, stats=ws[f"st2_{i}"][:T], H=H)
                nxt = {}
                if fuse_ln and i + 1 < nb:
                    nxt = dict(ln_out=ws[f"Q{i + 1}"][:T], ln_w=P.view(f"attention_layernorms.{i + 1}.weight"),
                               ln_b=P.view(f"attention_layernorms.{i + 1}.bias"), ln_eps=LN_EPS,
                               ln_stats=ws[f"st1_{i + 1}"][:T])
                if self.fuse_ffn and Hp <= 128:
                    ops.mlp2_tn(y, self.sh[f"w1{i}"], self.sh[f"w2{i}"], h1, x[i + 1], bias1=self.bias("b1", i),
                                bias2=self.bias("b2", i), relu1=True, drop1_p=p_drop, drop2_p=p_drop, drop1_stream=11 + 4 * i,
                                drop2_stream=12 + 4 * i, drop_seed=seed, drop_step=step, residual_is_a=True, row_ids=row_ids,
                                **nxt)
                else:
                    ops.gemm_tn(y, self.sh[f"w1{i}"], out_bf16=h1, bias=self.bias("b1", i), relu=True,
                                drop_p=p_drop, drop_seed=seed, drop_stream=11 + 4 * i, drop_step=step)
                    ops.gemm_tn(h1, self.sh[f"w2{i}"], out_bf16=x[i + 1], bias=self.bias("b2", i), residual=y, row_ids=row_ids,
                                drop_p=p_drop, drop_seed=seed, drop_stream=12 + 4 * i, drop_step=step, **nxt)
            fin_in = x[nb]
            if s.kind == "SRFR":
                ops.gemm_tn(x[nb], self.sh["wc"], out_bf16=ws["c"][:T], bias=self.bias("bc"))
                fin_in = ws["c"][:T]
            if not last_only:
                ops.layernorm_fwd(fin_in, P.view("last_layernorm.weight"), P.view("last_layernorm.bias"), LN_EPS,
                                  y_f32=ws["hfin"][:T], stats=ws["stF"][:T], H=s.Dout)
        if last_only:
            out = ws["hfin"][:B]
            ops.layernorm_fwd_rows(fin_in, P.view("last_layernorm.weight"), P.view("last_layernorm.bias"), LN_EPS, out,
                                   plan.last_row, B, s.Dout)
            return out[:, :s.Dout]
        if training if save is None else save:
            self.saved = dict(seq=seq, aux_ids=aux_ids, B=B, L=L, p_drop=p_drop, seed=seed, step=step,
                              version=self.fwd_version, plan=plan, hyb=hyb, live=live)
        return ws["hfin"][:T]

    def _fuse_oproj(self, hyb, L, fuse_ln) -> int:
        s = self.spec
        if hyb is not None or s.num_heads != 1 or not fuse_ln or s.Hp != s.H:
            return 0
        return ops.attention_packed_oproj_supported(L, s.H, s.num_heads)

    def _backward_packed(self, dh: torch.Tensor) -> None:
        s, P, sv = self.spec, self.P, self.saved
        plan, hyb, live = sv["plan"], sv.get("hyb"), sv.get("live")
        B, L = sv["B"], sv["L"]
        T, H, Hp, nb = plan.cap, s.H, s.Hp, s.num_blocks
        ws = self._ws
        row_ids = plan.row_ids
        p_drop, seed, step = sv["p_drop"], sv["seed"], sv["step"]
        gA, gC, gD, gX = (ws[n][:T] for n in ("gA", "gC", "gD", "gX"))
        G = lambda name: P.view(name, grad=True)
        GM = lambda name: P.mat(name, grad=True)
        x = [ws[f"x{i}"][:T] for i in range(nb + 1)]
        dz_top = ws[f"gdz_{nb - 1}"][:T]
        fuse_oproj = self._fuse_oproj(hyb, L, Hp <= 128 and os.environ.get("SRFRD_FUSE_LN", "1") != "0") & 2
        with ops.row_limit(plan.rows):
            if s.kind == "SRFR":
                gc = ws["gc"][:T]
                ops.layernorm_bwd(dh, ws["c"][:T], ws["stF"][:T], P.view("last_layernorm.weight"), gc,
                                  G("last_layernorm.weight"), G("last_layernorm.bias"), H=s.D)
                with self._branch():
                    ops.gemm_wgrad(gc, x[nb], GM("last_conv.weight"), G("last_conv.bias"), Mo=s.D, No=H)
                ops.gemm_tn(gc, self.sh["wcT"], out_bf16=dz_top, row_ids=row_ids)
            else:
                ops.layernorm_bwd(dh, x[nb], ws["stF"][:T], P.view("last_layernorm.weight"), dz_top,
                                  G("last_layernorm.weight"), G("last_layernorm.bias"), row_ids=row_ids, H=s.Dout)
            for i in reversed(range(nb)):
                Q, q, kv, o, r, y, h1 = (ws[f"{n}{i}"][:T] for n in ("Q", "q", "kv", "o", "r", "y", "h1"))
                dz, da1, dr, dq, dkv = (ws[f"{n}{i}"][:T] for n in ("gdz_", "gda1_", "gdr_", "gdq_", "gdkv_"))
                dx_out = ws[f"gdz_{i - 1}"][:T] if i > 0 else gA
                dz2 = dz
                if p_drop > 0:
                    dz2 = ws[f"gE_{i}"][:T]
                    ops.dropout_apply(dz, dz2, Hp, p_drop, seed, 12 + 4 * i, step)
                with self._branch():
                    ops.gemm_wgrad(dz2, h1, GM(f"forward_layers.{i}.conv2.weight"), G(f"forward_layers.{i}.conv2.bias"), Mo=H, No=H)
                if self.fuse_ffn and Hp <= 128:
                    ops.mlp2_tn(dz2, self.sh[f"w2T{i}"], self.sh[f"w1T{i}"], da1, gC, gate=h1, drop1_p=p_drop,
                                drop1_stream=11 + 4 * i, drop_seed=seed, drop_step=step, residual=dz)
                    with self._branch():
                        ops.gemm_wgrad(da1, y, GM(f"forward_layers.{i}.conv1.weight"), G(f"forward_layers.{i}.conv1.bias"),
                                       Mo=H, No=H)
                else:
                    ops.gemm_tn(dz2, self.sh[f"w2T{i}"], out_bf16=da1, gate=h1, drop_p=p_drop, drop_seed=seed,
                                drop_stream=11 + 4 * i, drop_step=step)
                    with self._branch():
                        ops.gemm_wgrad(da1, y, GM(f"forward_layers.{i}.conv1.weight"), G(f"forward_layers.{i}.conv1.bias"),
                                       Mo=H, No=H)
                    ops.gemm_tn(da1, self.sh[f"w1T{i}"], out_bf16=gC, residual=dz)
                ops.layernorm_bwd(gC, r, ws[f"st2_{i}"][:T], P.view(f"forward_layernorms.{i}.weight"), dr,
                                  G(f"forward_layernorms.{i}.weight"), G(f"forward_layernorms.{i}.bias"), H=H)
                with self._branch():
                    ops.gemm_wgrad(dr, o, GM(f"attention_layers.{i}.out_proj.weight"),
                                   G(f"attention_layers.{i}.out_proj.bias"), Mo=H, No=H)
                if not fuse_oproj:
                    ops.gemm_tn(dr, self.sh[f"woT{i}"], out_bf16=gC)
                if fuse_oproj:
                    ops.attention_bwd_packed(None, q, kv[:, :Hp], kv[:, Hp:], dq, dkv[:, :Hp], dkv[:, Hp:], plan, L, H,
                                             s.num_heads, p_drop, seed, 10 + 4 * i, step, dr=dr, woT=self.sh[f"woT{i}"])
                elif hyb is None:
                    ops.attention_bwd_packed(gC, q, kv[:, :Hp], kv[:, Hp:], dq, dkv[:, :Hp], dkv[:, Hp:], plan, L, H,
                                             s.num_heads, p_drop, seed, 10 + 4 * i, step)
                else:
                    Td = B * L
                    qd, kvd, od = hyb[f"qd{i}"][:Td], hyb[f"kvd{i}"][:Td], hyb[f"od{i}"][:Td]
                    dod, dqd, dkvd = hyb["dod"][:Td], hyb["dqd"][:Td], hyb["dkvd"][:Td]
                    ops.unpack_rows([(gC, dod, Hp, 1)], plan)
                    with (live.active() if live is not None else nullcontext()):
                        ops.attention_bwd(dod, qd, kvd[:, :Hp], kvd[:, Hp:], dqd, dkvd[:, :Hp], dkvd[:, Hp:], B, L, H,
                                          s.num_heads, p_drop, seed, 10 + 4 * i, step, o=od, stats=ws.get(f"ast{i}"))
                    ops.pack_rows([(dqd, dq, Hp, 0), (dkvd, dkv, 2 * Hp, 1)], plan)
                gin = GM(f"attention_layers.{i}.in_proj_weight")
                gbin = G(f"attention_layers.{i}.in_proj_bias")
                with self._branch():
                    ops.gemm_wgrad(dq, Q, gin[:H], gbin[:H], Mo=H, No=H)
                    ops.gemm_wgrad(dkv, x[i], gin[H:], gbin[H:], Mo=2 * H, No=H)
                with self._branch(second=True):
                    ops.gemm_tn(dkv, self.sh[f"wkvT{i}"], out_bf16=gX)
                ops.gemm_tn(dq, self.sh[f"wqT{i}"], out_bf16=gD, residual=dr)
                self._join(second=True)
                ops.layernorm_bwd(gD, x[i], ws[f"st1_{i}"][:T], P.view(f"attention_layernorms.{i}.weight"), dx_out,
                                  G(f"attention_layernorms.{i}.weight"), G(f"attention_layernorms.{i}.bias"),
                                  add=gX, row_ids=row_ids, H=H)
            dx0 = gA
            if s.kind == "SASRec" and p_drop > 0:
                ops.dropout_apply(gA, gC, H, p_drop, seed, 1, step)
                dx0 = gC
        aux_grad = G(s.aux_key) if s.aux_key else None
        ops.embed_bwd_packed(dx0, sv["seq"], sv["aux_ids"], plan, s.D, s.F if s.mode == 1 else 0, s.mode, s.item_scale,
                             G(s.item_key), aux_grad, G(s.pos_key))
        self._join()
        self.saved = None

    def fake_table(self) -> Optional[torch.Tensor]:
        return self.P.view("embedding_layer.fake_embed.weight") if self.spec.kind == "SRFRN" else None

    def fake_table_grad(self) -> Optional[torch.Tensor]:
        return self.P.view("embedding_layer.fake_embed.weight", grad=True) if self.spec.kind == "SRFRN" else None
```

srfrd_b200/ops.py:

```python
from __future__ import annotations

import ctypes as C
from typing import Optional

import torch

from . import _lib
from contextlib import contextmanager

from ._lib import CastDesc, GemmEpilogue, Mlp2Epilogue, PackDesc, RepackPart, call

bf16 = torch.bfloat16


def _p(t: Optional[torch.Tensor]):
    return None if t is None else t.data_ptr()


def _stream():
    return torch.cuda.current_stream().cuda_stream


def _chk(t: torch.Tensor, dtype, name: str):
    if not t.is_cuda:
        raise RuntimeError(f"srfrd_b200: {name} must be a CUDA tensor (there is no CPU fallback)")
    if t.dtype != dtype:
        raise RuntimeError(f"srfrd_b200: {name} must be {dtype}, got {t.dtype}")
    if t.stride(-1) != 1:
        raise RuntimeError(f"srfrd_b200: {name} must be contiguous in its last dimension")


def embed_ln_fwd(item_table, pos_table, aux_table, mode, seq, aux_ids, item_scale, ln_w, ln_b, eps,
                 x0_bf16=None, x0_f32=None, q_bf16=None, stats=None, drop_p=0.0, drop_seed=0, drop_stream=0,
                 drop_step=None):
    _lib.require_device()
    B, L = seq.shape
    D = item_table.shape[1]
    F = aux_table.shape[1] if (aux_table is not None and mode == 1) else 0
    _chk(item_table, torch.float32, "item_table"); _chk(seq, torch.int64, "seq")
    ldx = (x0_bf16 if x0_bf16 is not None else q_bf16).stride(0) if (x0_bf16 is not None or q_bf16 is not None) else D + F
    call("srfrd_embed_ln_fwd", _p(item_table), item_table.shape[0], D, _p(pos_table), _p(aux_table),
         0 if aux_table is None else aux_table.shape[0], F, mode, _p(seq), _p(aux_ids), B, L, float(item_scale),
         _p(ln_w), _p(ln_b), float(eps), _p(x0_bf16), _p(x0_f32), _p(q_bf16), _p(stats), ldx, float(drop_p),
         int(drop_seed), int(drop_stream), _p(drop_step), _stream())


def srfu_labels(fake_ids, kind: int, labels):
    _lib.require_device()
    B, L = fake_ids.shape
    call("srfrd_srfu_labels", _p(fake_ids), B, L, kind, _p(labels), _stream())


def embed_bwd(dx0, seq, aux_ids, D, F, mode, item_scale, d_item, d_aux):
    B, L = seq.shape
    call("srfrd_embed_bwd", _p(dx0), dx0.stride(0), _p(seq), _p(aux_ids), B, L, D, F, mode, float(item_scale),
         _p(d_item), _p(d_aux), _stream())


def layernorm_fwd(x, w, b, eps, y_bf16=None, y_f32=None, stats=None, T=None, H=None, row_stride=1, row_offset=0):
    _lib.require_device()
    T = x.shape[0] if T is None else T
    H = x.shape[1] if H is None else H
    y = y_bf16 if y_bf16 is not None else y_f32
    call("srfrd_layernorm_fwd", _p(x), x.stride(0), _p(w), _p(b), float(eps), _p(y_bf16), _p(y_f32), y.stride(0),
         _p(stats), T, H, row_stride, row_offset, _stream())


def layernorm_bwd(dy, x, stats, w, dx, dw, db, add=None, row_ids=None, H=None):
    T = x.shape[0]
    H = x.shape[1] if H is None else H
    dyb = dy if dy.dtype == bf16 else None
    dyf = dy if dy.dtype == torch.float32 else None
    call("srfrd_layernorm_bwd", _p(dyb), _p(dyf), dy.stride(0), _p(x), x.stride(0), _p(stats), _p(w), _p(add),
         0 if add is None else add.stride(0), _p(row_ids), _p(dx), dx.stride(0), _p(dw), _p(db), T, H, _stream())


def gemm_tn(A, B, out_bf16=None, out_f32=None, bias=None, residual=None, gate=None, row_ids=None, relu=False,
            drop_p=0.0, drop_seed=0, drop_stream=0, drop_step=None, M=None, ln_out=None, ln_w=None, ln_b=None, ln_eps=0.0,
            ln_stats=None):
    _lib.require_device()
    M = A.shape[0] if M is None else M
    K = A.shape[1]
    N = B.shape[0]
    out = out_bf16 if out_bf16 is not None else out_f32
    ep = GemmEpilogue(_p(bias), _p(residual), _p(gate), _p(row_ids), _p(out_bf16), _p(out_f32),
                      0 if residual is None else residual.stride(0), 0 if gate is None else gate.stride(0),
                      out.stride(0), int(relu), float(drop_p), int(drop_stream), int(drop_seed), _p(drop_step),
                      _p(ln_out), _p(ln_w), _p(ln_b), _p(ln_stats), 0 if ln_out is None else ln_out.stride(0), float(ln_eps))
    call("srfrd_gemm_tn", _p(A), A.stride(0), _p(B), B.stride(0), M, N, K, C.byref(ep), _stream())


def gemm_wgrad(dY, X, dW, dbias=None, Mo=None, No=None):
    T = dY.shape[0]
    Mo = dY.shape[1] if Mo is None else Mo
    No = X.shape[1] if No is None else No
    call("srfrd_gemm_wgrad", _p(dY), dY.stride(0), _p(X), X.stride(0), T, Mo, No, _p(dW), dW.stride(0), _p(dbias),
         _stream())


def gemm_ref(A, B, Cout, a_mn_major=False, b_mn_major=False):
    _lib.require_device()
    M, N = Cout.shape
    K = A.shape[0] if a_mn_major else A.shape[1]
    call("srfrd_gemm_ref", _p(A), A.stride(0), _p(B), B.stride(0), _p(Cout), Cout.stride(0), M, N, K,
         int(a_mn_major), int(b_mn_major), _stream())


def colsum(X, out, M=None, N=None, ld=None):
    M = X.shape[0] if M is None else M
    N = X.shape[1] if N is None else N
    ld = X.stride(0) if ld is None else ld
    call("srfrd_colsum", _p(X), M, N, ld, _p(out), _stream())


def add_segments(src, n, seg_in, seg_out, out):
    call("srfrd_add_segments", _p(src), n, seg_in, seg_out, _p(out), _stream())


def dropout_apply(x, out, N, drop_p, seed, stream_id, drop_step=None):
    call("srfrd_dropout_apply", _p(x), x.stride(0), _p(out), out.stride(0), x.shape[0], N, float(drop_p), int(seed),
         int(stream_id), _p(drop_step), _stream())


def cast_weights(descs_dev, n):
    call("srfrd_cast_weights", _p(descs_dev), n, _stream())


def make_cast_table(entries, device):
    arr = (CastDesc * len(entries))()
    for i, (src, dst, dst_t) in enumerate(entries):
        is_f32 = int(dst is not None and dst.dtype == torch.float32)
        arr[i] = CastDesc(src.data_ptr(), src.stride(0), _p(dst), 0 if dst is None else dst.stride(0), _p(dst_t),
                          0 if dst_t is None else dst_t.stride(0), src.shape[0], src.shape[1], is_f32)
    raw = bytes(arr)
    host = torch.frombuffer(bytearray(raw), dtype=torch.uint8)
    return host.to(device), len(entries)


def f32_to_bf16_split(src, hi, lo=None, row_index=None):
    _lib.require_device()
    rows = src.shape[0] if row_index is None else row_index.numel()
    cols = src.shape[1]
    call("srfrd_f32_to_bf16_split", _p(src), src.stride(0), _p(row_index), _p(hi), _p(lo), rows, cols, hi.stride(0),
         _stream())


def attention_fwd(q, k, v, o, B, L, H, heads, drop_p=0.0, seed=0, stream_id=0, drop_step=None, stats=None):
    _lib.require_device()
    call("srfrd_attention_fwd", _p(q), q.stride(0), _p(k), _p(v), k.stride(0), _p(o), o.stride(0), _p(stats), B, L, H, heads,
         float(drop_p), int(seed), int(stream_id), _p(drop_step), _stream())


def attention_bwd(dout, q, k, v, dq, dk, dv, B, L, H, heads, drop_p=0.0, seed=0, stream_id=0, drop_step=None, o=None,
                  stats=None):
    call("srfrd_attention_bwd", _p(dout), dout.stride(0), _p(q), q.stride(0), _p(k), _p(v), k.stride(0), _p(o),
         0 if o is None else o.stride(0), _p(stats), _p(dq), dq.stride(0), _p(dk), _p(dv), dk.stride(0), B, L, H, heads,
         float(drop_p), int(seed), int(stream_id), _p(drop_step), _stream())


def score_fwd(h, item_table, fake_table, pos, neg, prs, nrs, zp, zn):
    _lib.require_device()
    T = pos.numel()
    D = item_table.shape[1]
    F = 0 if fake_table is None else fake_table.shape[1]
    call("srfrd_score_fwd", _p(h), h.stride(0), _p(item_table), _p(fake_table), _p(pos), _p(neg), _p(prs), _p(nrs), T,
         D, F, _p(zp), _p(zn), _stream())


def score_bwd(h, item_table, fake_table, pos, neg, prs, nrs, dzp, dzn, dh, d_item, d_fake):
    T = pos.numel()
    D = item_table.shape[1]
    F = 0 if fake_table is None else fake_table.shape[1]
    call("srfrd_score_bwd", _p(h), h.stride(0), _p(item_table), _p(fake_table), _p(pos), _p(neg), _p(prs), _p(nrs),
         _p(dzp), _p(dzn), T, D, F, _p(dh), dh.stride(0), _p(d_item), _p(d_fake), _stream())


def score_loss_fused(h, item_table, fake_table, pos, neg, prs, nrs, w_pos, w_neg, norm, loss_acc, dh, d_item, d_fake,
                     zp=None, zn=None):
    T = pos.numel()
    D = item_table.shape[1]
    F = 0 if fake_table is None else fake_table.shape[1]
    call("srfrd_score_loss_fused", _p(h), h.stride(0), _p(item_table), _p(fake_table), _p(pos), _p(neg), _p(prs),
         _p(nrs), _p(w_pos), _p(w_neg), _p(norm), T, D, F, _p(zp), _p(zn), _p(loss_acc), _p(dh),
         0 if dh is None else dh.stride(0), _p(d_item), _p(d_fake), _stream())


def weight_sums(pos, w_pos, w_neg, out2):
    _lib.require_device()
    call("srfrd_weight_sums", _p(pos), _p(w_pos), _p(w_neg), pos.numel(), _p(out2), _stream())


def loss_finalize(acc2, norm2, loss):
    call("srfrd_loss_finalize", _p(acc2), _p(norm2), _p(loss), _stream())


def adam_tick(state3, beta1, beta2):
    call("srfrd_adam_tick", _p(state3), float(beta1), float(beta2), _stream())


def adam_step(p, g, m, v, lr, beta1, beta2, eps, state3, zero_grad=True):
    _lib.require_device()
    call("srfrd_adam_step", _p(p), _p(g), _p(m), _p(v), p.numel(), float(lr), float(beta1), float(beta2), float(eps),
         _p(state3), int(zero_grad), _stream())


def adam_step_fused(p, g, m, v, lr, beta1, beta2, eps, state8, zero_grad=True, acc2=None, norm2=None, loss=None,
                    l2: Optional["ParamL2"] = None):
    _lib.require_device()
    call("srfrd_adam_step_fused", _p(p), _p(g), _p(m), _p(v), p.numel(), float(lr), float(beta1), float(beta2), float(eps),
         _p(state8), int(zero_grad), _p(acc2), _p(norm2), _p(loss), _stream(), *_l2_args(l2))


class ParamL2:

    def __init__(self, segments, l2: float, device):
        host = (C.c_int64 * (2 * len(segments)))(*[int(x) for s in segments for x in s])
        n_chunks = C.c_int64(0)
        call("srfrd_param_l2_plan", host, len(segments), C.byref(n_chunks))
        self.n_seg, self.n_chunks, self.l2 = len(segments), int(n_chunks.value), float(l2)
        self.seg = torch.tensor([int(x) for s in segments for x in s], dtype=torch.int64).to(device)
        self.coef = torch.zeros(self.n_seg, dtype=torch.float32, device=device)
        self.reg = torch.zeros(1, dtype=torch.float32, device=device)
        self.ws = torch.zeros(self.n_chunks + 1, dtype=torch.float64, device=device)

    def launch(self, p: torch.Tensor):
        _lib.require_device()
        _chk(p, torch.float32, "p")
        call("srfrd_param_l2", _p(p), _p(self.seg), self.n_seg, self.n_chunks, self.l2, _p(self.coef), _p(self.reg),
             _p(self.ws), _stream())


def _l2_args(l2: Optional[ParamL2]):
    return (None, 0, None, None) if l2 is None else (_p(l2.seg), l2.n_seg, _p(l2.coef), _p(l2.reg))


def catalogue_topk_plan(U, n_rows, row_lo, D, n_split, k=10) -> int:
    out = C.c_int(0)
    call("srfrd_catalogue_topk_plan", U, n_rows, row_lo, D, n_split, C.byref(out), int(k))
    return out.value


def catalogue_topk_kmax(D, n_split) -> int:
    out = C.c_int(0)
    call("srfrd_catalogue_topk_kmax", D, n_split, C.byref(out))
    return out.value


def catalogue_topk(feats, U, u_pad, n_split, table, row_lo, id_base, chunks, part_scores, part_ids, packed=None, k=10):
    _lib.require_device()
    D = table.shape[1]
    call("srfrd_catalogue_topk", _p(feats), U, u_pad, n_split, _p(table), table.shape[0], row_lo, id_base, D,
         feats.stride(0), table.stride(0), chunks, _p(part_scores), _p(part_ids), _p(packed), _stream(), int(k))


def catalogue_rank(feats, U, u_pad, n_split, table, row_lo, id_base, target_rows, target_ids, rank_out,
                   target_scores=None):
    _lib.require_device()
    D = table.shape[1]
    call("srfrd_catalogue_rank", _p(feats), U, u_pad, n_split, _p(table), table.shape[0], row_lo, id_base, D,
         feats.stride(0), table.stride(0), _p(target_rows), target_rows.stride(0), _p(target_ids), _p(target_scores),
         _p(rank_out), _stream())


def merge_topk_packed(packed, U, nlists, k, out_scores, out_ids):
    _lib.require_device()
    call("srfrd_merge_topk_packed", _p(packed), U, nlists, k, _p(out_scores), _p(out_ids), _stream())


def merge_topk(scores, ids, U, nlists, k, out_scores, out_ids):
    _lib.require_device()
    call("srfrd_merge_topk", _p(scores), _p(ids), U, nlists, k, _p(out_scores), _p(out_ids), _stream())


def sample_batch(offsets, items, labels, p_fake, eligible, itemnum, B, L, policy, seed, step, out, w_pos=None):
    _lib.require_device()
    call("srfrd_sample_batch", _p(offsets), _p(items), _p(labels), _p(p_fake), _p(eligible), eligible.numel(), int(itemnum),
         B, L, int(policy), int(seed), _p(step), _p(out.get("users")), _p(out["seq"]), _p(out["rsq"]), _p(out["pos"]),
         _p(out["prs"]), _p(out["neg"]), _p(out["nrs"]), _p(w_pos), _stream())


def sample_candidates(offsets, items, users0, target, itemnum, C, seed, cand):
    _lib.require_device()
    call("srfrd_sample_candidates", _p(offsets), _p(items), _p(users0), _p(target), users0.numel(), int(itemnum), int(C),
         int(seed), _p(cand), _stream())


def candidate_rank(feats, item_table, cand, D, fake_table=None, user_label=None, logits=None, rank=None, err_flag=None):
    _lib.require_device()
    _chk(feats, torch.float32, "feats"); _chk(item_table, torch.float32, "item_table"); _chk(cand, torch.int64, "cand")
    U, Cn = cand.shape
    F = 0 if fake_table is None else fake_table.shape[1]
    call("srfrd_candidate_rank", _p(feats), feats.stride(0), _p(item_table), item_table.shape[0], int(D), _p(cand), U, Cn,
         _p(fake_table), F, _p(user_label), _p(logits), 0 if logits is None else logits.stride(0), _p(rank), _p(err_flag),
         _stream())


def add_user_term(logits, feats_tail, fake_table, label):
    _lib.require_device()
    U, I = logits.shape
    call("srfrd_add_user_term", _p(logits), logits.stride(0), U, I, _p(feats_tail), feats_tail.stride(0), _p(fake_table),
         _p(label), fake_table.shape[1], _stream())


class PackedPlan:

    def __init__(self, B: int, L: int, device):
        self.B, self.L = B, L
        self.cap = (B * (L + 1) + 127) // 128 * 128
        i32 = lambda n: torch.zeros(n, dtype=torch.int32, device=device)
        self.rows, self.cnt, self.seq_first = i32(4), i32(B), i32(B + 1)
        self.tok_row, self.row_tok = i32(B * L), i32(self.cap)
        self.row_ids = torch.zeros(self.cap, dtype=torch.int64, device=device)
        self.row_info = i32(4 * self.cap)
        self.tile_row0, self.last_row = i32(B + 130), i32(B)
        self.desc = PackDesc(_p(self.rows), _p(self.cnt), _p(self.seq_first), _p(self.tok_row), _p(self.row_tok),
                             _p(self.row_ids), _p(self.row_info), _p(self.tile_row0), _p(self.last_row), self.cap)

    def build(self, seq, keep=None):
        _lib.require_device()
        B, L = seq.shape
        assert (B, L) == (self.B, self.L)
        _chk(seq, torch.int64, "seq")
        call("srfrd_pack_plan", _p(seq), _p(keep), B, L, C.byref(self.desc), _stream())


@contextmanager
def row_limit(rows_dev):
    call("srfrd_set_row_limit", _p(rows_dev))
    try:
        yield
    finally:
        call("srfrd_set_row_limit", None)


class LiveTiles:

    def __init__(self, B: int, L: int, heads: int, device):
        nq = (L + 127) // 128
        self.B, self.L, self.heads = B, L, heads
        self.q_lo = torch.zeros(B, dtype=torch.int32, device=device)
        self.items = torch.zeros(B * heads * nq, dtype=torch.int32, device=device)
        self.n_live = torch.zeros(1, dtype=torch.int32, device=device)

    def build(self, plan: "PackedPlan"):
        _lib.require_device()
        assert (plan.B, plan.L) == (self.B, self.L)
        self.tok_row = plan.tok_row
        call("srfrd_attention_live_items", _p(plan.tok_row), self.B, self.L, self.heads, _p(self.q_lo), _p(self.items),
             _p(self.n_live), _stream())

    @contextmanager
    def active(self):
        call("srfrd_set_attention_live", _p(self.q_lo), _p(self.items), _p(self.n_live), _p(self.tok_row))
        try:
            yield
        finally:
            call("srfrd_set_attention_live", None, None, None, None)


def attention_packed_supported(L: int, H: int, heads: int) -> bool:
    return bool(_lib.load().srfrd_attention_packed_supported(int(L), int(H), int(heads)))


def embed_ln_fwd_packed(item_table, pos_table, aux_table, mode, seq, aux_ids, item_scale, ln_w, ln_b, eps, x0_bf16, q_bf16,
                        stats, plan: PackedPlan, drop_p=0.0, drop_seed=0, drop_stream=0, drop_step=None):
    _lib.require_device()
    B, L = seq.shape
    D = item_table.shape[1]
    F = aux_table.shape[1] if (aux_table is not None and mode == 1) else 0
    call("srfrd_embed_ln_fwd_packed", _p(item_table), item_table.shape[0], D, _p(pos_table), _p(aux_table),
         0 if aux_table is None else aux_table.shape[0], F, mode, _p(seq), _p(aux_ids), B, L, float(item_scale), _p(ln_w),
         _p(ln_b), float(eps), _p(x0_bf16), _p(q_bf16), _p(stats), x0_bf16.stride(0), float(drop_p), int(drop_seed),
         int(drop_stream), _p(drop_step), _p(plan.row_tok), _p(plan.rows), plan.cap, _stream())


def layernorm_fwd_rows(x, w, b, eps, y_f32, row_index, n, H):
    _lib.require_device()
    call("srfrd_layernorm_fwd_rows", _p(x), x.stride(0), _p(w), _p(b), float(eps), _p(y_f32), y_f32.stride(0), _p(row_index),
         n, H, _stream())


def attention_packed_oproj_supported(L: int, H: int, heads: int) -> int:
    return int(_lib.load().srfrd_attention_packed_oproj_supported(int(L), int(H), int(heads)))


def attention_fwd_packed(q, k, v, o, plan: PackedPlan, L, H, heads, drop_p=0.0, seed=0, stream_id=0, drop_step=None,
                         wo=None, bias=None, residual=None, r=None, y=None, ln_w=None, ln_b=None, ln_eps=0.0, ln_stats=None):
    _lib.require_device()
    st = lambda t: 0 if t is None else t.stride(0)
    call("srfrd_attention_fwd_packed", _p(q), q.stride(0), _p(k), _p(v), k.stride(0), _p(o), o.stride(0), C.byref(plan.desc),
         L, H, heads, float(drop_p), int(seed), int(stream_id), _p(drop_step), _stream(), _p(wo), st(wo), _p(bias),
         _p(residual), st(residual), _p(ln_w), _p(ln_b), float(ln_eps), _p(ln_stats), _p(r), st(r), _p(y), st(y))


def attention_bwd_packed(dout, q, k, v, dq, dk, dv, plan: PackedPlan, L, H, heads, drop_p=0.0, seed=0, stream_id=0,
                         drop_step=None, dr=None, woT=None):
    st = lambda t: 0 if t is None else t.stride(0)
    call("srfrd_attention_bwd_packed", _p(dout), st(dout), _p(q), q.stride(0), _p(k), _p(v), k.stride(0), _p(dq),
         dq.stride(0), _p(dk), _p(dv), dk.stride(0), C.byref(plan.desc), L, H, heads, float(drop_p), int(seed),
         int(stream_id), _p(drop_step), _stream(), _p(dr), st(dr), _p(woT), st(woT))


def score_loss_fused_packed(h, item_table, fake_table, pos, neg, prs, nrs, w_pos, w_neg, norm, loss_acc, dh, d_item, d_fake,
                            plan: PackedPlan):
    D = item_table.shape[1]
    F = 0 if fake_table is None else fake_table.shape[1]
    call("srfrd_score_loss_fused_packed", _p(h), h.stride(0), _p(item_table), _p(fake_table), _p(pos), _p(neg), _p(prs),
         _p(nrs), _p(w_pos), _p(w_neg), _p(norm), D, F, _p(loss_acc), _p(dh), dh.stride(0), _p(d_item), _p(d_fake),
         _p(plan.row_tok), _p(plan.rows), plan.cap, _stream())


def embed_bwd_packed(dx0, seq, aux_ids, plan: PackedPlan, D, F, mode, item_scale, d_item, d_aux, d_pos):
    B, L = seq.shape
    call("srfrd_embed_bwd_packed", _p(dx0), dx0.stride(0), _p(seq), _p(aux_ids), _p(plan.row_tok), _p(plan.rows), plan.cap,
         L, D, F, mode, float(item_scale), _p(d_item), _p(d_aux), _p(d_pos), _stream())


def dp_adam_step(grad_ptrs_dev: int, param_ptrs_dev: int, signal_ptrs_dev: int, rank, world, n, m, v, lr, beta1, beta2, eps,
                 state8, norm2, local4, l2: Optional[ParamL2] = None):
    _lib.require_device()
    call("srfrd_dp_adam_step", grad_ptrs_dev, param_ptrs_dev, signal_ptrs_dev, int(rank), int(world), int(n), _p(m), _p(v),
         float(lr), float(beta1), float(beta2), float(eps), _p(state8), _p(norm2), _p(local4), _stream(), *_l2_args(l2))


def _parts(parts):
    arr = (RepackPart * len(parts))()
    for i, (src, dst, W, mode) in enumerate(parts):
        arr[i] = RepackPart(_p(src), src.stride(0), _p(dst), dst.stride(0), int(W), int(mode))
    return arr


def unpack_rows(parts, plan: PackedPlan):
    _lib.require_device()
    arr = _parts(parts)
    call("srfrd_unpack_rows", arr, len(parts), C.byref(plan.desc), plan.B, plan.L, _stream())


def pack_rows(parts, plan: PackedPlan):
    _lib.require_device()
    arr = _parts(parts)
    call("srfrd_pack_rows", arr, len(parts), C.byref(plan.desc), plan.B, plan.L, _stream())


def mlp2_tn(A, W1, W2, mid_out, out, bias1=None, bias2=None, gate=None, relu1=False, drop1_p=0.0, drop2_p=0.0, drop1_stream=0,
            drop2_stream=0, drop_seed=0, drop_step=None, residual=None, residual_is_a=False, row_ids=None, ln_out=None,
            ln_w=None, ln_b=None, ln_stats=None, ln_eps=0.0, M=None):
    _lib.require_device()
    M = A.shape[0] if M is None else M
    N = W1.shape[0]
    ep = Mlp2Epilogue(_p(bias1), _p(bias2), _p(gate), 0 if gate is None else gate.stride(0), int(relu1), float(drop1_p),
                      float(drop2_p), int(drop1_stream), int(drop2_stream), int(drop_seed), _p(drop_step), _p(residual),
                      0 if residual is None else residual.stride(0), int(residual_is_a), _p(row_ids), _p(mid_out),
                      mid_out.stride(0), _p(out), out.stride(0), _p(ln_out), 0 if ln_out is None else ln_out.stride(0),
                      _p(ln_w), _p(ln_b), _p(ln_stats), float(ln_eps))
    call("srfrd_mlp2_tn", _p(A), A.stride(0), _p(W1), W1.stride(0), _p(W2), W2.stride(0), M, N, C.byref(ep), _stream())


def catalogue_ce_plan(Dp: int):
    smem, stages, tmem = C.c_int64(0), C.c_int(0), C.c_int(0)
    call("srfrd_catalogue_ce_plan", int(Dp), C.byref(smem), C.byref(stages), C.byref(tmem))
    return int(smem.value), int(stages.value), int(tmem.value)


def _ce_rows(h, plan):
    return (None, None, h.shape[0]) if plan is None else (plan.row_tok, plan.rows, plan.cap)


def catalogue_ce_fwd(h, table, pos, w_pos, lse, loss_acc, plan: Optional[PackedPlan] = None):
    _lib.require_device()
    _chk(h, bf16, "h"); _chk(table, bf16, "table"); _chk(pos, torch.int64, "pos")
    row_tok, rows, cap = _ce_rows(h, plan)
    call("srfrd_catalogue_ce_fwd", _p(h), h.stride(0), _p(table), table.stride(0), table.shape[0] - 1, table.shape[1],
         _p(pos), _p(w_pos), _p(row_tok), _p(rows), cap, _p(lse), _p(loss_acc), _stream())


def catalogue_ce_bwd(h, table, pos, w_pos, norm, lse, dh, d_item, D, plan: Optional[PackedPlan] = None):
    _lib.require_device()
    _chk(h, bf16, "h"); _chk(table, bf16, "table"); _chk(pos, torch.int64, "pos")
    row_tok, rows, cap = _ce_rows(h, plan)
    call("srfrd_catalogue_ce_bwd", _p(h), h.stride(0), _p(table), table.stride(0), table.shape[0] - 1, table.shape[1],
         int(D), _p(pos), _p(w_pos), _p(norm), _p(row_tok), _p(rows), cap, _p(lse), _p(dh),
         0 if dh is None else dh.stride(0), _p(d_item), 0 if d_item is None else d_item.stride(0), _stream())
```

srfrd_b200/trainer.py:

```python
from __future__ import annotations

import time
from typing import Dict, Optional

import numpy as np
import torch

from . import ops, parallel
from .engine import HotPath
from .losses import check_ce_width

__all__ = ["simulate", "FusedTrainer", "DeviceSampler", "discriminator_weights"]

POLICIES = {"none": 0, "mask": 1, "soft": 2}


class DeviceSampler:

    def __init__(self, data, maxlen: int, device, seed: int = 0):
        dev = torch.device(device)
        self.L, self.itemnum, self.seed = maxlen, int(data.itemnum), int(seed)
        self.offsets = torch.as_tensor(np.asarray(data.offsets, np.int64)).to(dev)
        self.items = torch.as_tensor(np.asarray(data.items, np.int32)).to(dev)
        self.labels = torch.as_tensor(np.asarray(data.labels, np.int8)).to(dev)
        pf = getattr(data, "p_fake", None)
        self.p_fake = None if pf is None else torch.as_tensor(np.asarray(pf, np.float32)).to(dev)
        lens = np.diff(np.asarray(data.offsets, np.int64))
        self.eligible = torch.as_tensor(np.nonzero(lens > 1)[0].astype(np.int32)).to(dev)
        if self.eligible.numel() == 0:
            raise ValueError("no user has more than one training interaction")
        self.device = dev
        self.draws = 0

    def alloc(self, B: int):
        z = lambda: torch.zeros(B, self.L, dtype=torch.int64, device=self.device)
        return dict(users=torch.zeros(B, dtype=torch.int64, device=self.device), seq=z(), rsq=z(), pos=z(), prs=z(),
                    neg=z(), nrs=z())

    def sample_into(self, out, w_pos=None, policy: str = "none", step=None):
        B = out["seq"].shape[0]
        ops.sample_batch(self.offsets, self.items, self.labels, self.p_fake, self.eligible, self.itemnum, B, self.L,
                         POLICIES[policy], self.seed + (0 if step is not None else self.draws), step, out, w_pos)
        self.draws += 1

    def next_batch(self, batch_size: int):
        out = self.alloc(batch_size)
        self.sample_into(out)
        return out["users"], out["seq"], out["rsq"], out["pos"], out["prs"], out["neg"], out["nrs"]



def discriminator_weights(pos: torch.Tensor, p_fake: Optional[torch.Tensor], policy: str = "none") -> torch.Tensor:
    valid = (pos != 0).to(torch.float32)
    if policy == "none" or p_fake is None:
        return valid
    if policy == "mask":
        return valid * (p_fake < 0.5).to(torch.float32)
    if policy == "soft":
        return valid * (1.0 - p_fake.to(torch.float32))
    raise ValueError(f"unknown discriminator weighting policy {policy!r}")


class FusedTrainer:

    def __init__(self, model, lr: float = 1e-3, betas=(0.9, 0.98), eps: float = 1e-8, process_group=None,
                 use_graph: bool = True, l2_emb: float = 0.0, packed: Optional[bool] = None, loss: str = "bce"):
        if loss not in ("bce", "ce"):
            raise ValueError(f"unknown loss {loss!r} (expected 'bce' or 'ce')")
        if loss == "ce":
            if model.spec.kind == "SRFRN":
                raise ValueError("loss='ce' does not support SRFRN: its logits need each candidate's fake label "
                                 "(SRFR_model.py:225-233), which unobserved items do not have")
            check_ce_width(model.spec.D)
        self.loss_kind = loss
        self.model = model
        self._dp = None
        if process_group is not None and torch.distributed.get_world_size(process_group) > 1:
            self._dp = self._setup_fused_dp(model, process_group)
        self.eng: HotPath = model._sync_flat()
        self.P = self.eng.P
        self.spec = self.eng.spec
        self.lr, self.betas, self.eps = lr, betas, eps
        self.pg = process_group
        self.use_graph = use_graph
        self.packed = self.eng.packed_default if packed is None else bool(packed)
        dev = self.eng.device
        self.m = torch.zeros_like(self.P.data)
        self.v = torch.zeros_like(self.P.data)
        self.scal = torch.zeros(8, dtype=torch.float32, device=dev)
        self.comm = torch.cuda.Stream(device=dev)
        self._static: Optional[Dict[str, torch.Tensor]] = None
        self._graph: Optional[torch.cuda.CUDAGraph] = None
        self._graph_key = None
        self._eager_key = None
        self._has_w = (False, False)
        self.l2_emb = float(l2_emb)
        self._l2 = self._setup_l2(model) if self.l2_emb != 0.0 else None
        self._ce_ws: Optional[Dict[str, torch.Tensor]] = None
        if loss == "ce":
            self.eng.enable_ce_table()
        self.P.grad_bucket.zero_()
        self.eng.refresh_shadows()
        self.steps = 0

    def _ce_buffers(self, rows: int) -> Dict[str, torch.Tensor]:
        if self._ce_ws is None or self._ce_ws["lse"].numel() < rows:
            dev = self.eng.device
            self._ce_ws = dict(h=torch.zeros(rows, self.spec.Dp, dtype=torch.bfloat16, device=dev),
                               lse=torch.zeros(rows, dtype=torch.float32, device=dev))
            self.eng.ws_generation += 1
        return self._ce_ws

    def _refuse_w_neg(self, w_neg):
        if w_neg is not None and self.loss_kind == "ce":
            raise ValueError("w_neg weights the sampled negatives of the BCE; loss='ce' has no negatives")

    def _setup_l2(self, model) -> ops.ParamL2:
        segs = self.P.segments()
        base = self.P.data.data_ptr()
        mine = sorted((p.data_ptr(), p.numel()) for p in model.parameters())
        assert mine == [(base + 4 * off, n) for off, n in segs], \
            "srfrd_b200: l2_emb: the flat parameter segments do not cover exactly model.parameters()"
        return ops.ParamL2(segs, self.l2_emb, self.eng.device)

    @staticmethod
    def _setup_fused_dp(model, pg):
        import os
        if os.environ.get("SRFRD_FUSED_DP", "1") == "0":
            return None
        try:
            import torch.distributed._symmetric_memory as symm
            dev = next(model.parameters()).device
            gname = pg.group_name
            try:
                symm.enable_symm_mem_for_group(gname)
            except Exception:
                pass
            eng = model.rehome(lambda n: symm.empty(n, dtype=torch.float32, device=dev))
            P = eng.P
            sig = symm.empty(64, dtype=torch.int32, device=dev).zero_()
            torch.cuda.synchronize()
            hg, hp, hs = (symm.rendezvous(t, gname) for t in (P.grad_bucket, P.data_ext, sig))
            dp = dict(g=int(hg.buffer_ptrs_dev), p=int(hp.buffer_ptrs_dev), s=int(hs.buffer_ptrs_dev), rank=int(hg.rank),
                      world=int(hg.world_size), keep=(hg, hp, hs, sig),
                      local=torch.zeros(4, dtype=torch.int32, device=dev))
            torch.cuda.synchronize()
            torch.distributed.barrier(group=pg)
            return dp
        except Exception as ex:
            import warnings
            warnings.warn(f"srfrd_b200: fused data-parallel optimizer unavailable ({type(ex).__name__}: {ex}); "
                          "falling back to the NCCL all-reduce + replicated Adam")
            return None

    @property
    def loss_dev(self) -> torch.Tensor:
        return self.P.data_tail[0] if self._dp is not None else self.scal[4]

    _KEYS = ("seq", "rsq", "pos", "prs", "neg", "nrs")

    @staticmethod
    def _carve(flat: torch.Tensor, B: int, L: int):
        n = B * L
        out = {k: flat[i * n:(i + 1) * n].view(B, L) for i, k in enumerate(FusedTrainer._KEYS)}
        w = flat[6 * n:7 * n].view(torch.float32)
        out["w_pos"], out["w_neg"] = w[:n].view(B, L), w[n:].view(B, L)
        return out

    def _alloc_static(self, B: int, L: int):
        dev = self.eng.device
        self._static_flat = torch.zeros(7 * B * L, dtype=torch.int64, device=dev)
        self._static = self._carve(self._static_flat, B, L)
        self._stage_flat = None
        self._graph = None

    def _step_body(self, has_wp: bool, has_wn: bool):
        st, eng, P, s = self._static, self.eng, self.P, self.spec
        B, L = st["seq"].shape
        T = B * L
        pos, neg = st["pos"].view(-1), st["neg"].view(-1)
        w_pos = st["w_pos"].view(-1) if has_wp else None
        w_neg = st["w_neg"].view(-1) if has_wn else None
        norm, acc, loss = self.scal[0:2], P.grad_tail[0:2], self.scal[4:5]
        smp = getattr(self, "_sampler", None)
        if smp is not None:
            smp.sample_into(st, st["w_pos"] if has_wp else None, self._sampler_policy, step=eng.step_state[3:4])
        self.comm.wait_stream(torch.cuda.current_stream())
        with torch.cuda.stream(self.comm):
            ops.weight_sums(pos, w_pos, w_neg, norm)
            if self.pg is not None:
                parallel.allreduce_sum_(norm, self.pg)
            if self._l2 is not None:
                self._l2.launch(P.data)
        packed = self.packed and eng.packed_ok(B, L)
        hidden = eng.forward(st["seq"], st["rsq"], training=True, packed=packed, keep=st["pos"] if packed else None)
        ws = eng._ws
        ft = eng.fake_table()
        torch.cuda.current_stream().wait_stream(self.comm)
        prs_ = st["prs"].view(-1) if ft is not None else None
        nrs_ = st["nrs"].view(-1) if ft is not None else None
        if self.loss_kind == "ce":
            plan = eng.saved["plan"] if packed else None
            rows = plan.cap if packed else T
            ce = self._ce_buffers(rows)
            hb, lse, table = ce["h"][:rows], ce["lse"][:rows], eng.sh["ce_table"]
            ops.f32_to_bf16_split(ws["hfin"][:rows], hb)
            ops.catalogue_ce_fwd(hb, table, pos, w_pos, lse, acc, plan)
            ops.catalogue_ce_bwd(hb, table, pos, w_pos, norm, lse, ws["dh"][:rows], P.view(s.item_key, grad=True), s.D, plan)
            eng.backward(ws["dh"][:rows])
        elif packed:
            plan = eng.saved["plan"]
            Tp = plan.cap
            ops.score_loss_fused_packed(ws["hfin"][:Tp], P.view(s.item_key), ft, pos, neg, prs_, nrs_, w_pos, w_neg, norm, acc,
                                        ws["dh"][:Tp], P.view(s.item_key, grad=True), eng.fake_table_grad(), plan)
            eng.backward(ws["dh"][:Tp])
        else:
            ops.score_loss_fused(ws["hfin"][:T], P.view(s.item_key), ft, pos, neg, prs_, nrs_, w_pos, w_neg, norm, acc,
                                 ws["dh"][:T], P.view(s.item_key, grad=True), eng.fake_table_grad())
            eng.backward(ws["dh"][:T])
        if self._dp is not None:
            d = self._dp
            ops.dp_adam_step(d["g"], d["p"], d["s"], d["rank"], d["world"], P.numel, self.m, self.v, self.lr, self.betas[0],
                             self.betas[1], self.eps, eng.step_state, norm, d["local"], l2=self._l2)
        else:
            if self.pg is not None:
                parallel.allreduce_sum_(P.grad_bucket, self.pg)
            ops.adam_step_fused(P.data, P.grad, self.m, self.v, self.lr, self.betas[0], self.betas[1], self.eps,
                                eng.step_state, zero_grad=True, acc2=acc, norm2=norm, loss=loss, l2=self._l2)
        eng.refresh_shadows()

    def load_batch(self, batch: Dict[str, torch.Tensor], w_pos=None, w_neg=None, non_blocking: bool = True):
        self._refuse_w_neg(w_neg)
        B, L = batch["seq"].shape
        if self._static is None or self._static["seq"].shape != (B, L):
            self._alloc_static(B, L)
        st = self._static
        for k in ("seq", "rsq", "pos", "prs", "neg", "nrs"):
            src = batch.get(k)
            if src is None:
                st[k].zero_()
            else:
                st[k].copy_(torch.as_tensor(src), non_blocking=non_blocking)
        if w_pos is not None:
            st["w_pos"].copy_(torch.as_tensor(w_pos), non_blocking=non_blocking)
        if w_neg is not None:
            st["w_neg"].copy_(torch.as_tensor(w_neg), non_blocking=non_blocking)
        self._has_w = (w_pos is not None, w_neg is not None)

    def pack_batch(self, batch: Dict[str, torch.Tensor], w_pos=None, w_neg=None) -> torch.Tensor:
        self._refuse_w_neg(w_neg)
        B, L = batch["seq"].shape
        flat = torch.zeros(7 * B * L, dtype=torch.int64, device=self.eng.device)
        v = self._carve(flat, B, L)
        for k in self._KEYS:
            if batch.get(k) is not None:
                v[k].copy_(torch.as_tensor(batch[k]))
        if w_pos is not None:
            v["w_pos"].copy_(torch.as_tensor(w_pos))
        if w_neg is not None:
            v["w_neg"].copy_(torch.as_tensor(w_neg))
        flat._srfrd_shape, flat._srfrd_w = (B, L), (w_pos is not None, w_neg is not None)
        return flat

    def step_packed(self, flat: torch.Tensor) -> torch.Tensor:
        B, L = flat._srfrd_shape
        if self._static is None or self._static["seq"].shape != (B, L):
            self._alloc_static(B, L)
        self._static_flat.copy_(flat, non_blocking=True)
        self._has_w = flat._srfrd_w
        return self.run_step()

    def prefetch(self, batch: Dict[str, torch.Tensor], w_pos=None, w_neg=None):
        self._refuse_w_neg(w_neg)
        B, L = batch["seq"].shape
        if self._static is None or self._static["seq"].shape != (B, L):
            self._alloc_static(B, L)
        if self._stage_flat is None:
            self._stage_flat = torch.zeros_like(self._static_flat)
            self._stage = self._carve(self._stage_flat, B, L)
            self._copy_stream = torch.cuda.Stream(device=self.eng.device)
            self._stage_free = torch.cuda.Event()
            self._stage_full = torch.cuda.Event()
            self._stage_free.record()
        with torch.cuda.stream(self._copy_stream):
            self._copy_stream.wait_event(self._stage_free)
            for k in self._KEYS:
                src = batch.get(k)
                if src is None:
                    self._stage[k].zero_()
                else:
                    self._stage[k].copy_(torch.as_tensor(src), non_blocking=True)
            if w_pos is not None:
                self._stage["w_pos"].copy_(torch.as_tensor(w_pos), non_blocking=True)
            if w_neg is not None:
                self._stage["w_neg"].copy_(torch.as_tensor(w_neg), non_blocking=True)
            self._stage_full.record()
        self._stage_w = (w_pos is not None, w_neg is not None)

    def step_prefetched(self) -> torch.Tensor:
        main = torch.cuda.current_stream()
        main.wait_event(self._stage_full)
        self._static_flat.copy_(self._stage_flat)
        self._stage_free.record(main)
        self._has_w = self._stage_w
        return self.run_step()

    def run_step(self) -> torch.Tensor:
        key = (tuple(self._static["seq"].shape), self._has_w, id(getattr(self, "_sampler", None)), self.eng.ws_generation)
        if self.use_graph and self._graph is not None and self._graph_key == key:
            self._graph.replay()
        elif self.use_graph and self.steps >= 1 and self._eager_key == key[:3] + (self.eng.ws_generation,):
            g = torch.cuda.CUDAGraph()
            torch.cuda.synchronize()
            with torch.cuda.graph(g):
                self._step_body(*self._has_w)
            self._graph, self._graph_key = g, key
            g.replay()
        else:
            self._step_body(*self._has_w)
            self._eager_key = key[:3] + (self.eng.ws_generation,)
        self.steps += 1
        return self.loss_dev

    def step(self, batch, w_pos=None, w_neg=None) -> torch.Tensor:
        self.load_batch(batch, w_pos, w_neg)
        return self.run_step()

    def step_sampled(self, sampler: "DeviceSampler", batch_size: int, policy: str = "none") -> torch.Tensor:
        if self._static is None or self._static["seq"].shape != (batch_size, sampler.L):
            self._alloc_static(batch_size, sampler.L)
        self._sampler, self._sampler_policy = sampler, policy
        self._has_w = (policy != "none", False)
        out = self.run_step()
        self._sampler = None
        return out

    def state_dict(self):
        return {k: v.detach().clone() for k, v in self.model.state_dict().items()}


def simulate(model, optimizer, criterion, sampler, config, wandb=None, model_index=0, num_batch=None, device=None,
             dataset=None, evaluation=None, log_every: int = 1):
    T, t0 = 0.0, time.time()
    metricsbyepoch = dict()
    device = device if device is not None else next(model.parameters()).device
    num_batch = num_batch if num_batch is not None else getattr(config, "num_batch")
    for epoch in range(config.num_epochs):
        if config.inference_only:
            break
        epoch_loss = 0.0
        model.train()
        for step in range(num_batch):
            u, seq, rsq, pos, prs, neg, nrs = sampler.next_batch()
            seq, rsq, pos, prs, neg, nrs = (torch.as_tensor(np.array(a)).long().to(device)
                                            for a in (seq, rsq, pos, prs, neg, nrs))
            hidden_state, pos_logits, neg_logits = model(user_ids=None, input_ids=seq, fake_ids=rsq, positive_ids=pos,
                                                         positive_fake_ids=prs, negative_ids=neg, negative_fake_ids=nrs)
            pos_labels = torch.ones(pos_logits.shape, device=device)
            neg_labels = torch.zeros(neg_logits.shape, device=device)
            optimizer.zero_grad()
            indices = torch.where(pos != 0)
            loss = criterion(pos_logits[indices], pos_labels[indices])
            loss += criterion(neg_logits[indices], neg_labels[indices])
            if getattr(config, "l2_emb", 0.0):
                for param in model.parameters():
                    loss += config.l2_emb * torch.norm(param)
            loss.backward()
            optimizer.step()
            if step % log_every == 0:
                li = loss.item()
                if wandb is not None:
                    wandb.log({"Training Loss by iteration": li})
                epoch_loss += li
        if wandb is not None:
            wandb.log({"Training Loss by Epoch": epoch_loss, "Epochs": epoch + 1})
        if (epoch + 1) % 10 == 0 and evaluation is not None and dataset is not None:
            model.eval()
            T += time.time() - t0
            t_test = evaluation(model, dataset, config.maxlen, device)
            if wandb is not None:
                wandb.log({"NDCG@10": t_test[0], "HT@10": t_test[1]})
            metricsbyepoch[epoch + 1] = {"NDCG@10": t_test[0], "HT@10": t_test[1]}
            t0 = time.time()
            model.train()
    return metricsbyepoch
```

Measured before the change: 9.821 million.

## Fuse final LayerNorm backward into score loss kernel and overlap shadow weight casts

Adds a score-loss kernel variant that also computes the final LayerNorm backward (input gradient plus weight and bias gradients) in one pass, so the separate dh write, read and layernorm_bwd launch are removed. It also moves the bf16 shadow-weight cast from the end of the step to the start of the next one, running on a side stream that overlaps weight_sums, and has the CE path write the bf16 hidden state directly from layernorm instead of running a separate conversion. In exchange the LN variant is capped to fewer blocks and uses more registers and shared atomics, and the lazy shadow refresh adds state that must stay consistent across graph replays.

```diff
diff --git a/include/srfrd_b200.h b/include/srfrd_b200.h
--- a/include/srfrd_b200.h
+++ b/include/srfrd_b200.h
@@ -8,7 +8,7 @@
 extern "C" {
 #endif
 
-#define SRFRD_ABI_VERSION 10
+#define SRFRD_ABI_VERSION 11
 #if defined(__GNUC__)
 #define SRFRD_API __attribute__((visibility("default")))
 #else
@@ -200,6 +200,12 @@
                                   const float* w_pos, const float* w_neg, const float* norm, int D, int F,
                                   float* loss_acc, float* dh, int lddh, float* d_item, float* d_fake,
                                   const int* row_tok, const int* rows_dev, int64_t cap_rows, void* stream);
+SRFRD_API int srfrd_score_loss_ln_bwd(const float* h, int ldh, const void* x, int ldx, const float* stats, const float* ln_w,
+                            const float* item_table, const float* fake_table, const int64_t* pos, const int64_t* neg,
+                            const int64_t* prs, const int64_t* nrs, const float* w_pos, const float* w_neg,
+                            const float* norm, int64_t T, int D, int F, float* loss_acc, void* gx, int ldgx,
+                            const int64_t* row_ids, float* d_ln_w, float* d_ln_b, float* d_item, float* d_fake,
+                            const int* row_tok, const int* rows_dev, void* stream);
 SRFRD_API int srfrd_embed_bwd_packed(const void* dx0_bf16, int ldx, const int64_t* seq, const int64_t* aux_ids,
                            const int* row_tok, const int* rows_dev, int64_t cap_rows, int L, int D, int F, int mode,
                            float item_scale, float* d_item, float* d_aux, float* d_pos, void* stream);
diff --git a/srfrd_b200/_lib.py b/srfrd_b200/_lib.py
--- a/srfrd_b200/_lib.py
+++ b/srfrd_b200/_lib.py
@@ -98,6 +98,8 @@
                                    f32, u64, u32, vp, vp, vp, i32, vp, i32],
     "srfrd_score_loss_fused_packed": [vp, i32, vp, vp, vp, vp, vp, vp, vp, vp, vp, i32, i32, vp, vp, i32, vp, vp, vp, vp,
                                       i64, vp],
+    "srfrd_score_loss_ln_bwd": [vp, i32, vp, i32, vp, vp, vp, vp, vp, vp, vp, vp, vp, vp, vp, i64, i32, i32, vp, vp, i32,
+                                vp, vp, vp, vp, vp, vp, vp, vp],
     "srfrd_embed_bwd_packed": [vp, i32, vp, vp, vp, vp, i64, i32, i32, i32, i32, f32, vp, vp, vp, vp],
     "srfrd_sample_candidates": [vp, vp, vp, vp, i64, i32, i32, u64, vp, vp],
     "srfrd_candidate_rank": [vp, i32, vp, i64, i32, vp, i64, i32, vp, i32, vp, vp, i32, vp, vp, vp],
@@ -125,7 +127,7 @@
         fn = getattr(lib, name)
         fn.argtypes = argtypes
         fn.restype = C.c_int
-    if lib.srfrd_abi_version() != 10:
+    if lib.srfrd_abi_version() != 11:
         raise RuntimeError("srfrd_b200: ABI version mismatch between _lib.py and the built library")
     _lib = lib
     return lib
diff --git a/srfrd_b200/csrc/loss_scatter_adam.cu b/srfrd_b200/csrc/loss_scatter_adam.cu
--- a/srfrd_b200/csrc/loss_scatter_adam.cu
+++ b/srfrd_b200/csrc/loss_scatter_adam.cu
@@ -4,6 +4,7 @@
 namespace srfrd {
 
 static constexpr int MAXC = 16;
+static constexpr int MAXC_LN = 8;
 
 struct ScoreParams {
   const float* h; int ldh;
@@ -22,18 +23,36 @@
   const int* row_tok;
   const int* rows_dev;
   int group;
+  const bf16* x; int ldx;
+  const float* stats;
+  const float* ln_w;
+  bf16* gx; int ldgx;
+  const int64_t* row_ids;
+  float *ln_dw, *ln_db;
 };
 
 __device__ __forceinline__ float softplus(float x) { return fmaxf(x, 0.f) + log1pf(__expf(-fabsf(x))); }
 __device__ __forceinline__ float sigmoidf(float x) { return 1.f / (1.f + __expf(-x)); }
 
-template <int NC>
-__global__ void __launch_bounds__(256, (NC <= 9 ? 2 : 1)) score_kernel(ScoreParams p) {
+template <int NC, bool LN>
+__global__ void __launch_bounds__(256, ((LN ? NC <= 2 : NC <= 9) ? 2 : 1)) score_kernel(ScoreParams p) {
   __shared__ float red[2][8];
+  __shared__ float sln[LN ? 2 * 32 * NC : 1];
   pdl_prologue_done();
   const int lane = threadIdx.x & 31, warp = threadIdx.x >> 5, nw = blockDim.x >> 5;
+  const int W = p.D + (p.fake_table ? p.F : 0);
+  float lw[LN ? NC : 1], adw[LN ? NC : 1], adb[LN ? NC : 1];
+  if constexpr (LN) {
+    for (int i = threadIdx.x; i < 2 * 32 * NC; i += blockDim.x) sln[i] = 0.f;
+#pragma unroll
+    for (int i = 0; i < NC; ++i) {
+      const int c = lane + 32 * i;
+      lw[i] = c < W ? __ldg(p.ln_w + c) : 0.f;
+      adw[i] = adb[i] = 0.f;
+    }
+    __syncthreads();
+  }
   const int64_t warp0 = (int64_t)blockIdx.x * nw + warp, nwarps = (int64_t)gridDim.x * nw;
-  const int W = p.D + (p.fake_table ? p.F : 0);
   float lp_acc = 0.f, ln_acc = 0.f;
   float inv_np = 0.f, inv_nn = 0.f;
   if (p.mode == 1) {
@@ -45,6 +64,8 @@
 #pragma unroll
   for (int i = 0; i < NC; ++i) fk1[i] = fk2[i] = 0.f;
   const bool dh_vec = p.dh && (p.lddh == W) && (W % 4 == 0) && ((reinterpret_cast<uintptr_t>(p.dh) & 15) == 0);
+  const bool gx_vec = LN && (p.ldgx == W) && (W % 8 == 0) && ((reinterpret_cast<uintptr_t>(p.gx) & 15) == 0);
+  const float invW = 1.f / (float)W;
   if (p.rows_dev) p.T = min(p.T, (int64_t)__ldg(p.rows_dev));
   const int G = p.group;
   for (int64_t t0 = warp0 * G; t0 < p.T; t0 += nwarps * G) {
@@ -56,6 +77,10 @@
     int64_t my_pid = 0, my_nid = 0, my_pf = 0, my_nf = 0;
     float my_a = 0.f, my_b = 0.f;
     bool my_active = false;
+    bool my_keep = true;
+    float2 my_st = make_float2(0.f, 0.f);
+    if (LN && in && p.row_ids) my_keep = __ldg(p.row_ids + tl) != 0;
+    if (LN && in) my_st = __ldg(reinterpret_cast<const float2*>(p.stats) + tl);
     if (in) {
       my_pid = __ldg(p.pos + my_src);
       my_nid = __ldg(p.neg + my_src);
@@ -73,6 +98,20 @@
       if (p.fake_table && my_active) { my_pf = __ldg(p.prs + my_src); my_nf = __ldg(p.nrs + my_src); }
     }
     unsigned mask = __ballot_sync(0xffffffffu, my_active);
+    if (LN) {
+      const int nrow = (int)min((int64_t)G, p.T - t0);
+      if (gx_vec) {
+        const int per_row = W >> 3, total = nrow * per_row;
+        uint4* base = reinterpret_cast<uint4*>(p.gx + t0 * p.ldgx);
+        for (int i = lane; i < total; i += 32)
+          if (!((mask >> (i / per_row)) & 1u)) base[i] = make_uint4(0, 0, 0, 0);
+      } else {
+        for (int r = 0; r < nrow; ++r) {
+          if ((mask >> r) & 1u) continue;
+          for (int c = lane; c < W; c += 32) p.gx[(t0 + r) * p.ldgx + c] = f2bf(0.f);
+        }
+      }
+    }
     if (p.dh) {
       const int nrow = (int)min((int64_t)G, p.T - t0);
       if (dh_vec) {
@@ -88,8 +127,8 @@
       }
     }
     struct Tok {
-      int64_t t, tsrc, pid, nid; int pf, nf; float ta, tb;
-      float hv[NC], ep[NC], en[NC];
+      int64_t t, tsrc, pid, nid; int pf, nf; float ta, tb; bool keep; float mean, rstd;
+      float hv[NC], ep[NC], en[NC], xv[LN ? NC : 1];
     };
     auto fetch = [&](Tok& k, int r) {
       k.t = t0 + r;
@@ -97,10 +136,15 @@
       k.pid = __shfl_sync(0xffffffffu, my_pid, r); k.nid = __shfl_sync(0xffffffffu, my_nid, r);
       k.pf = (int)__shfl_sync(0xffffffffu, (int)my_pf, r); k.nf = (int)__shfl_sync(0xffffffffu, (int)my_nf, r);
       k.ta = __shfl_sync(0xffffffffu, my_a, r); k.tb = __shfl_sync(0xffffffffu, my_b, r);
+      if (LN) {
+        k.keep = __shfl_sync(0xffffffffu, my_keep, r);
+        k.mean = __shfl_sync(0xffffffffu, my_st.x, r); k.rstd = __shfl_sync(0xffffffffu, my_st.y, r);
+      }
 #pragma unroll
       for (int i = 0; i < NC; ++i) {
         const int c = lane + 32 * i;
         k.hv[i] = k.ep[i] = k.en[i] = 0.f;
+        if (LN) k.xv[LN ? i : 0] = c < W ? bf2f(p.x[k.t * p.ldx + c]) : 0.f;
         if (c < W) {
           k.hv[i] = p.h[k.t * p.ldh + c];
           if (c < p.D) {
@@ -126,6 +170,28 @@
         ln_acc += k.tb * softplus(zn);
         dzp = k.ta * (sigmoidf(zp) - 1.f) * inv_np;
         dzn = k.tb * sigmoidf(zn) * inv_nn;
+      }
+      if constexpr (LN) {
+        const float a = k.rstd, nb = -k.mean * k.rstd;
+        float dh[NC], xh[NC], sg = 0.f, sgx = 0.f;
+#pragma unroll
+        for (int i = 0; i < NC; ++i) {
+          xh[i] = fmaf(k.xv[i], a, nb);
+          dh[i] = dzp * k.ep[i] + dzn * k.en[i];
+          const float g = dh[i] * lw[i];
+          adw[i] = fmaf(dh[i], xh[i], adw[i]);
+          adb[i] += dh[i];
+          sg += g;
+          sgx = fmaf(g, xh[i], sgx);
+        }
+        sg = warp_sum(sg) * invW;
+        sgx = warp_sum(sgx) * invW;
+#pragma unroll
+        for (int i = 0; i < NC; ++i) {
+          const int c = lane + 32 * i;
+          const float u = fmaf(-sgx, xh[i], fmaf(dh[i], lw[i], -sg));
+          if (c < W) p.gx[k.t * p.ldgx + c] = f2bf(k.keep ? a * u : 0.f);
+        }
       }
 #pragma unroll
       for (int i = 0; i < NC; ++i) {
@@ -173,6 +239,18 @@
         if (fk1[i] != 0.f) red_add_f32(p.d_fake + 1 * p.F + (c - p.D), fk1[i]);
         if (fk2[i] != 0.f) red_add_f32(p.d_fake + 2 * p.F + (c - p.D), fk2[i]);
       }
+    }
+  }
+  if constexpr (LN) {
+#pragma unroll
+    for (int i = 0; i < NC; ++i) {
+      const int c = lane + 32 * i;
+      if (c < W) { atomicAdd(&sln[c], adw[i]); atomicAdd(&sln[32 * NC + c], adb[i]); }
+    }
+    __syncthreads();
+    for (int c = threadIdx.x; c < W; c += blockDim.x) {
+      if (sln[c] != 0.f) red_add_f32(p.ln_dw + c, sln[c]);
+      if (sln[32 * NC + c] != 0.f) red_add_f32(p.ln_db + c, sln[32 * NC + c]);
     }
   }
   if (p.mode == 1 && p.loss_acc) {
@@ -519,15 +597,25 @@
 
 static int score_launch(ScoreParams& p, void* stream) {
   const int W = p.D + (p.fake_table ? p.F : 0);
-  SRFRD_REQUIRE(W <= 32 * MAXC, "score: width %d unsupported", W);
+  const bool ln = p.x != nullptr;
+  SRFRD_REQUIRE(W <= 32 * (ln ? MAXC_LN : MAXC), "score: width %d unsupported", W);
   if (p.T == 0) return 0;
   if (p.group != 8) p.group = 32;
   int64_t blocks = (p.T + 8 * p.group - 1) / (8 * p.group);
-  const int64_t cap = (int64_t)num_sms() * 8;
+  const int64_t cap = (int64_t)num_sms() * (ln ? 2 : 8);
   if (blocks > cap) blocks = cap;
   const int nc = (W + 31) / 32;
-#define SCORE_CALL(NC) SRFRD_CUDA(launch_pdl(score_kernel<NC>, dim3((unsigned)blocks), dim3(256), 0, (cudaStream_t)stream, p))
-  if (nc <= 1) SCORE_CALL(1);
+#define SCORE_CALL(NC) SRFRD_CUDA(launch_pdl(score_kernel<NC, false>, dim3((unsigned)blocks), dim3(256), 0, (cudaStream_t)stream, p))
+#define SCORE_LN_CALL(NC) SRFRD_CUDA(launch_pdl(score_kernel<NC, true>, dim3((unsigned)blocks), dim3(256), 0, (cudaStream_t)stream, p))
+  if (ln) {
+    if (nc <= 1) SCORE_LN_CALL(1);
+    else if (nc <= 2) SCORE_LN_CALL(2);
+    else if (nc <= 3) SCORE_LN_CALL(3);
+    else if (nc <= 4) SCORE_LN_CALL(4);
+    else if (nc <= 6) SCORE_LN_CALL(6);
+    else SCORE_LN_CALL(MAXC_LN);
+  }
+  else if (nc <= 1) SCORE_CALL(1);
   else if (nc <= 2) SCORE_CALL(2);
   else if (nc <= 3) SCORE_CALL(3);
   else if (nc <= 4) SCORE_CALL(4);
@@ -535,6 +623,7 @@
   else if (nc <= 9) SCORE_CALL(9);
   else SCORE_CALL(MAXC);
 #undef SCORE_CALL
+#undef SCORE_LN_CALL
   SRFRD_LAUNCH_CHECK();
   return 0;
 }
@@ -590,6 +679,30 @@
   p.nrs = nrs; p.w_pos = w_pos; p.w_neg = w_neg; p.norm = norm; p.T = cap_rows; p.D = D; p.F = F;
   p.loss_acc = loss_acc; p.dh = dh; p.lddh = lddh; p.d_item = d_item; p.d_fake = d_fake; p.mode = 1;
   p.row_tok = row_tok; p.rows_dev = rows_dev; p.group = 8;
+  return score_launch(p, stream);
+}
+
+extern "C" int srfrd_score_loss_ln_bwd(const float* h, int ldh, const void* x, int ldx, const float* stats,
+                                         const float* ln_w, const float* item_table, const float* fake_table, const int64_t* pos,
+                                         const int64_t* neg, const int64_t* prs, const int64_t* nrs, const float* w_pos,
+                                         const float* w_neg, const float* norm, int64_t T, int D, int F, float* loss_acc,
+                                         void* gx, int ldgx, const int64_t* row_ids, float* d_ln_w, float* d_ln_b,
+                                         float* d_item, float* d_fake, const int* row_tok, const int* rows_dev,
+                                         void* stream) {
+  SRFRD_REQUIRE(h && x && stats && ln_w && item_table && pos && neg && norm && loss_acc && gx && d_ln_w && d_ln_b,
+                "score_loss_ln_bwd: null pointer");
+  SRFRD_REQUIRE(!fake_table || (prs && nrs), "score_loss_ln_bwd: fake ids required with a fake table");
+  SRFRD_REQUIRE((row_tok == nullptr) == (rows_dev == nullptr), "score_loss_ln_bwd: pass both row_tok and rows_dev or neither");
+  const int W = D + (fake_table ? F : 0);
+  SRFRD_REQUIRE(W >= 1 && ldh >= W && ldx >= W && ldgx >= W, "score_loss_ln_bwd: width %d / ld (%d, %d, %d) unsupported", W,
+                ldh, ldx, ldgx);
+  ScoreParams p = {};
+  p.item_table = item_table; p.fake_table = fake_table; p.pos = pos; p.neg = neg; p.prs = prs; p.nrs = nrs;
+  p.w_pos = w_pos; p.w_neg = w_neg; p.norm = norm; p.T = T; p.D = D; p.F = F; p.loss_acc = loss_acc;
+  p.d_item = d_item; p.d_fake = d_fake; p.mode = 1;
+  p.h = h; p.ldh = ldh; p.x = (const bf16*)x; p.ldx = ldx; p.stats = stats; p.ln_w = ln_w; p.gx = (bf16*)gx; p.ldgx = ldgx;
+  p.row_ids = row_ids; p.ln_dw = d_ln_w; p.ln_db = d_ln_b;
+  if (row_tok) { p.row_tok = row_tok; p.rows_dev = rows_dev; p.group = 8; }
   return score_launch(p, stream);
 }
 
diff --git a/srfrd_b200/engine.py b/srfrd_b200/engine.py
--- a/srfrd_b200/engine.py
+++ b/srfrd_b200/engine.py
@@ -207,7 +207,8 @@
             vec("bc", P.view("last_conv.bias"), Dp)
         self._cast_entries = entries
         self._cast_table, self._cast_n = ops.make_cast_table(entries, dev)
-        self.shadows_version = -1
+        self.shadows_stale = False
+        self._shadows_pending = False
 
     def enable_ce_table(self) -> torch.Tensor:
         if "ce_table" not in self.sh:
@@ -234,8 +235,19 @@
                "b2": f"forward_layers.{i}.conv2.bias"}[tag]
         return P.view(key)
 
-    def refresh_shadows(self):
-        ops.cast_weights(self._cast_table, self._cast_n)
+    def refresh_shadows(self, overlap: bool = False):
+        if overlap and self.overlap:
+            with self._branch(second=True):
+                ops.cast_weights(self._cast_table, self._cast_n)
+            self._shadows_pending = True
+        else:
+            ops.cast_weights(self._cast_table, self._cast_n)
+        self.shadows_stale = False
+
+    def _await_shadows(self):
+        if self._shadows_pending:
+            self._join(second=True)
+            self._shadows_pending = False
 
     @contextmanager
     def _branch(self, second: bool = False):
@@ -346,13 +358,15 @@
 
     def forward(self, seq: torch.Tensor, fake_ids: Optional[torch.Tensor], training: bool,
                 last_only: bool = False, save: Optional[bool] = None, packed: bool = False,
-                keep: Optional[torch.Tensor] = None) -> torch.Tensor:
+                keep: Optional[torch.Tensor] = None, hfin_bf16: Optional[torch.Tensor] = None) -> torch.Tensor:
         s, P = self.spec, self.P
         B, L = seq.shape
         if L > s.max_len:
             raise RuntimeError(f"sequence length {L} exceeds max_len {s.max_len} (pos_embed rows, SRFR_model.py:12)")
+        if self.shadows_stale:
+            self.refresh_shadows()
         if packed:
-            return self._forward_packed(seq, fake_ids, training, last_only, save, keep)
+            return self._forward_packed(seq, fake_ids, training, last_only, save, keep, hfin_bf16)
         T, H, Hp, nb = B * L, s.H, s.Hp, s.num_blocks
         ws = self._workspace(T, L)
         self.fwd_version += 1
@@ -378,6 +392,7 @@
                          drop_p=p_drop if s.kind == "SASRec" else 0.0, drop_seed=seed, drop_stream=1, drop_step=step)
         seq_flat = seq.view(-1)
         fuse_ln = (H == Hp) and Hp <= 128 and os.environ.get("SRFRD_FUSE_LN", "1") != "0"
+        self._await_shadows()
         for i in range(nb):
             Q, q, kv, o, r, y, h1 = (ws[f"{n}{i}"][:T] for n in ("Q", "q", "kv", "o", "r", "y", "h1"))
             with self._branch():
@@ -416,14 +431,19 @@
             ops.layernorm_fwd(fin_in, P.view("last_layernorm.weight"), P.view("last_layernorm.bias"), LN_EPS, y_f32=out,
                               T=B, H=s.Dout, row_stride=L, row_offset=L - 1)
             return out[:, :s.Dout]
-        ops.layernorm_fwd(fin_in, P.view("last_layernorm.weight"), P.view("last_layernorm.bias"), LN_EPS, y_f32=hfin,
-                          stats=ws["stF"][:T], H=s.Dout)
+        if hfin_bf16 is not None:
+            hfin = hfin_bf16[:T]
+            ops.layernorm_fwd(fin_in, P.view("last_layernorm.weight"), P.view("last_layernorm.bias"), LN_EPS, y_bf16=hfin,
+                              stats=ws["stF"][:T], H=s.Dout)
+        else:
+            ops.layernorm_fwd(fin_in, P.view("last_layernorm.weight"), P.view("last_layernorm.bias"), LN_EPS, y_f32=hfin,
+                              stats=ws["stF"][:T], H=s.Dout)
         if training if save is None else save:
             self.saved = dict(seq=seq, aux_ids=aux_ids, B=B, L=L, p_drop=p_drop, seed=seed, step=step,
-                              version=self.fwd_version)
-        return hfin.view(B, L, s.Doutp)[..., :s.Dout]
-
-    def backward(self, dh: torch.Tensor, version: Optional[int] = None) -> None:
+                              version=self.fwd_version, fin_in=fin_in, ln_bwd_done=False)
+        return hfin.view(B, L, -1)[..., :s.Dout]
+
+    def backward(self, dh: Optional[torch.Tensor], version: Optional[int] = None) -> None:
         s, P, sv = self.spec, self.P, self.saved
         if sv is None:
             raise RuntimeError("backward() without a training forward()")
@@ -431,6 +451,9 @@
             raise RuntimeError("srfrd_b200: backward() of a stale forward -- another forward() (training, validation or "
                                "predict) ran on this model after the one being back-propagated and overwrote the shared "
                                "activation workspace; run backward() before the next forward()")
+        if (dh is None) != sv["ln_bwd_done"]:
+            raise RuntimeError("srfrd_b200: backward(None) follows score_loss_ln_bwd(), and only it; otherwise pass "
+                               "dL/dhidden")
         if sv.get("plan") is not None:
             return self._backward_packed(dh)
         B, L = sv["B"], sv["L"]
@@ -446,12 +469,13 @@
 
         if s.kind == "SRFR":
             gc = ws["gc"][:T]
-            ops.layernorm_bwd(dh, ws["c"][:T], ws["stF"][:T], P.view("last_layernorm.weight"), gc,
-                              G("last_layernorm.weight"), G("last_layernorm.bias"), H=s.D)
+            if dh is not None:
+                ops.layernorm_bwd(dh, ws["c"][:T], ws["stF"][:T], P.view("last_layernorm.weight"), gc,
+                                  G("last_layernorm.weight"), G("last_layernorm.bias"), H=s.D)
             with self._branch():
                 ops.gemm_wgrad(gc, x[nb], GM("last_conv.weight"), G("last_conv.bias"), Mo=s.D, No=H)
             ops.gemm_tn(gc, self.sh["wcT"], out_bf16=dz_top, row_ids=seq_flat)
-        else:
+        elif dh is not None:
             ops.layernorm_bwd(dh, x[nb], ws["stF"][:T], P.view("last_layernorm.weight"), dz_top,
                               G("last_layernorm.weight"), G("last_layernorm.bias"), row_ids=seq_flat, H=s.Dout)
 
@@ -508,7 +532,7 @@
         self._join()
         self.saved = None
 
-    def _forward_packed(self, seq, fake_ids, training, last_only, save, keep):
+    def _forward_packed(self, seq, fake_ids, training, last_only, save, keep, hfin_bf16):
         s, P = self.spec, self.P
         B, L = seq.shape
         H, Hp, nb = s.H, s.Hp, s.num_blocks
@@ -546,6 +570,7 @@
                                     P.view("attention_layernorms.0.weight"), P.view("attention_layernorms.0.bias"), LN_EPS,
                                     x[0], ws["Q0"][:T], ws["st1_0"][:T], plan,
                                     drop_p=p_drop if s.kind == "SASRec" else 0.0, drop_seed=seed, drop_stream=1, drop_step=step)
+            self._await_shadows()
             for i in range(nb):
                 Q, q, kv, o, r, y, h1 = (ws[f"{n}{i}"][:T] for n in ("Q", "q", "kv", "o", "r", "y", "h1"))
                 with self._branch():
@@ -599,9 +624,11 @@
             if s.kind == "SRFR":
                 ops.gemm_tn(x[nb], self.sh["wc"], out_bf16=ws["c"][:T], bias=self.bias("bc"))
                 fin_in = ws["c"][:T]
+            hfin = ws["hfin"][:T] if hfin_bf16 is None else hfin_bf16[:T]
             if not last_only:
                 ops.layernorm_fwd(fin_in, P.view("last_layernorm.weight"), P.view("last_layernorm.bias"), LN_EPS,
-                                  y_f32=ws["hfin"][:T], stats=ws["stF"][:T], H=s.Dout)
+                                  y_f32=hfin if hfin_bf16 is None else None, y_bf16=None if hfin_bf16 is None else hfin,
+                                  stats=ws["stF"][:T], H=s.Dout)
         if last_only:
             out = ws["hfin"][:B]
             ops.layernorm_fwd_rows(fin_in, P.view("last_layernorm.weight"), P.view("last_layernorm.bias"), LN_EPS, out,
@@ -609,8 +636,8 @@
             return out[:, :s.Dout]
         if training if save is None else save:
             self.saved = dict(seq=seq, aux_ids=aux_ids, B=B, L=L, p_drop=p_drop, seed=seed, step=step,
-                              version=self.fwd_version, plan=plan, hyb=hyb, live=live)
-        return ws["hfin"][:T]
+                              version=self.fwd_version, plan=plan, hyb=hyb, live=live, fin_in=fin_in, ln_bwd_done=False)
+        return hfin
 
     def _fuse_oproj(self, hyb, L, fuse_ln) -> int:
         s = self.spec
@@ -635,12 +662,13 @@
         with ops.row_limit(plan.rows):
             if s.kind == "SRFR":
                 gc = ws["gc"][:T]
-                ops.layernorm_bwd(dh, ws["c"][:T], ws["stF"][:T], P.view("last_layernorm.weight"), gc,
-                                  G("last_layernorm.weight"), G("last_layernorm.bias"), H=s.D)
+                if dh is not None:
+                    ops.layernorm_bwd(dh, ws["c"][:T], ws["stF"][:T], P.view("last_layernorm.weight"), gc,
+                                      G("last_layernorm.weight"), G("last_layernorm.bias"), H=s.D)
                 with self._branch():
                     ops.gemm_wgrad(gc, x[nb], GM("last_conv.weight"), G("last_conv.bias"), Mo=s.D, No=H)
                 ops.gemm_tn(gc, self.sh["wcT"], out_bf16=dz_top, row_ids=row_ids)
-            else:
+            elif dh is not None:
                 ops.layernorm_bwd(dh, x[nb], ws["stF"][:T], P.view("last_layernorm.weight"), dz_top,
                                   G("last_layernorm.weight"), G("last_layernorm.bias"), row_ids=row_ids, H=s.Dout)
             for i in reversed(range(nb)):
@@ -710,6 +738,26 @@
         self._join()
         self.saved = None
 
+    def score_loss_ln_bwd(self, pos, neg, prs, nrs, w_pos, w_neg, norm, loss_acc) -> None:
+        s, P, sv = self.spec, self.P, self.saved
+        if sv is None or sv["version"] != self.fwd_version or sv["ln_bwd_done"]:
+            raise RuntimeError("srfrd_b200: score_loss_ln_bwd() needs the latest forward to be a training forward that "
+                               "has not been back-propagated")
+        plan = sv.get("plan")
+        x = sv["fin_in"]
+        rows = x.shape[0]
+        if s.kind == "SRFR":
+            gx, row_ids = self._ws["gc"][:rows], None
+        else:
+            gx = self._ws[f"gdz_{s.num_blocks - 1}"][:rows]
+            row_ids = plan.row_ids if plan is not None else sv["seq"].view(-1)
+        G = lambda name: P.view(name, grad=True)
+        ops.score_loss_ln_bwd(self._ws["hfin"][:rows], x, self._ws["stF"][:rows], P.view("last_layernorm.weight"),
+                              P.view(s.item_key), self.fake_table(), pos, neg, prs, nrs, w_pos, w_neg, norm, loss_acc, gx,
+                              G("last_layernorm.weight"), G("last_layernorm.bias"), G(s.item_key), self.fake_table_grad(),
+                              row_ids=row_ids, plan=plan)
+        sv["ln_bwd_done"] = True
+
     def fake_table(self) -> Optional[torch.Tensor]:
         return self.P.view("embedding_layer.fake_embed.weight") if self.spec.kind == "SRFRN" else None
 
diff --git a/srfrd_b200/ops.py b/srfrd_b200/ops.py
--- a/srfrd_b200/ops.py
+++ b/srfrd_b200/ops.py
@@ -410,6 +410,18 @@
          _p(plan.row_tok), _p(plan.rows), plan.cap, _stream())
 
 
+def score_loss_ln_bwd(h, x, stats, ln_w, item_table, fake_table, pos, neg, prs, nrs, w_pos, w_neg, norm, loss_acc, gx,
+                      d_ln_w, d_ln_b, d_item, d_fake, row_ids=None, plan: Optional[PackedPlan] = None):
+    _lib.require_device()
+    D = item_table.shape[1]
+    F = 0 if fake_table is None else fake_table.shape[1]
+    T = plan.cap if plan is not None else pos.numel()
+    call("srfrd_score_loss_ln_bwd", _p(h), h.stride(0), _p(x), x.stride(0), _p(stats), _p(ln_w), _p(item_table),
+         _p(fake_table), _p(pos), _p(neg), _p(prs), _p(nrs), _p(w_pos), _p(w_neg), _p(norm), T, D, F, _p(loss_acc), _p(gx),
+         gx.stride(0), _p(row_ids), _p(d_ln_w), _p(d_ln_b), _p(d_item), _p(d_fake),
+         None if plan is None else _p(plan.row_tok), None if plan is None else _p(plan.rows), _stream())
+
+
 def embed_bwd_packed(dx0, seq, aux_ids, plan: PackedPlan, D, F, mode, item_scale, d_item, d_aux, d_pos):
     B, L = seq.shape
     call("srfrd_embed_bwd_packed", _p(dx0), dx0.stride(0), _p(seq), _p(aux_ids), _p(plan.row_tok), _p(plan.rows), plan.cap,
diff --git a/srfrd_b200/trainer.py b/srfrd_b200/trainer.py
--- a/srfrd_b200/trainer.py
+++ b/srfrd_b200/trainer.py
@@ -186,6 +186,7 @@
         if smp is not None:
             smp.sample_into(st, st["w_pos"] if has_wp else None, self._sampler_policy, step=eng.step_state[3:4])
         self.comm.wait_stream(torch.cuda.current_stream())
+        eng.refresh_shadows(overlap=True)
         with torch.cuda.stream(self.comm):
             ops.weight_sums(pos, w_pos, w_neg, norm)
             if self.pg is not None:
@@ -193,7 +194,9 @@
             if self._l2 is not None:
                 self._l2.launch(P.data)
         packed = self.packed and eng.packed_ok(B, L)
-        hidden = eng.forward(st["seq"], st["rsq"], training=True, packed=packed, keep=st["pos"] if packed else None)
+        rows = eng._plan(B, L).cap if packed else T
+        hb = self._ce_buffers(rows)["h"][:rows] if self.loss_kind == "ce" else None
+        eng.forward(st["seq"], st["rsq"], training=True, packed=packed, keep=st["pos"] if packed else None, hfin_bf16=hb)
         ws = eng._ws
         ft = eng.fake_table()
         torch.cuda.current_stream().wait_stream(self.comm)
@@ -201,23 +204,13 @@
         nrs_ = st["nrs"].view(-1) if ft is not None else None
         if self.loss_kind == "ce":
             plan = eng.saved["plan"] if packed else None
-            rows = plan.cap if packed else T
-            ce = self._ce_buffers(rows)
-            hb, lse, table = ce["h"][:rows], ce["lse"][:rows], eng.sh["ce_table"]
-            ops.f32_to_bf16_split(ws["hfin"][:rows], hb)
+            lse, table = self._ce_ws["lse"][:rows], eng.sh["ce_table"]
             ops.catalogue_ce_fwd(hb, table, pos, w_pos, lse, acc, plan)
             ops.catalogue_ce_bwd(hb, table, pos, w_pos, norm, lse, ws["dh"][:rows], P.view(s.item_key, grad=True), s.D, plan)
             eng.backward(ws["dh"][:rows])
-        elif packed:
-            plan = eng.saved["plan"]
-            Tp = plan.cap
-            ops.score_loss_fused_packed(ws["hfin"][:Tp], P.view(s.item_key), ft, pos, neg, prs_, nrs_, w_pos, w_neg, norm, acc,
-                                        ws["dh"][:Tp], P.view(s.item_key, grad=True), eng.fake_table_grad(), plan)
-            eng.backward(ws["dh"][:Tp])
         else:
-            ops.score_loss_fused(ws["hfin"][:T], P.view(s.item_key), ft, pos, neg, prs_, nrs_, w_pos, w_neg, norm, acc,
-                                 ws["dh"][:T], P.view(s.item_key, grad=True), eng.fake_table_grad())
-            eng.backward(ws["dh"][:T])
+            eng.score_loss_ln_bwd(pos, neg, prs_, nrs_, w_pos, w_neg, norm, acc)
+            eng.backward(None)
         if self._dp is not None:
             d = self._dp
             ops.dp_adam_step(d["g"], d["p"], d["s"], d["rank"], d["world"], P.numel, self.m, self.v, self.lr, self.betas[0],
@@ -227,7 +220,6 @@
                 parallel.allreduce_sum_(P.grad_bucket, self.pg)
             ops.adam_step_fused(P.data, P.grad, self.m, self.v, self.lr, self.betas[0], self.betas[1], self.eps,
                                 eng.step_state, zero_grad=True, acc2=acc, norm2=norm, loss=loss, l2=self._l2)
-        eng.refresh_shadows()
 
     def load_batch(self, batch: Dict[str, torch.Tensor], w_pos=None, w_neg=None, non_blocking: bool = True):
         self._refuse_w_neg(w_neg)
@@ -319,6 +311,7 @@
         else:
             self._step_body(*self._has_w)
             self._eager_key = key[:3] + (self.eng.ws_generation,)
+        self.eng.shadows_stale = True
         self.steps += 1
         return self.loss_dev
 
```

Result: faster. 9.999 million, median of 6 (+1.8%).
